# fanxiaochen/Multi-View-Registration

Measured on NVIDIA B200. Metric: nn_queries_per_s (24-view x 200k turntable registration; ms_per_step = registration ms; a query = one PCL-equivalent nearest-neighbour answer: every source point per iteration + every gated match's reciprocal answer, the oracle's counter), higher is better.
Workload: dtype f32

## Files before the change

multi-view-registration_b200/csrc/api.cu:

```cuda
#include <cfloat>
#include <chrono>
#include <cstdlib>
#include <climits>
#include <cmath>
#include <cstdio>
#include <cstring>
#include <memory>
#include <string>
#include <thread>
#include <vector>

#include "../../include/mvr_b200.h"
#include "launch.h"
#include "small_solve.h"

#ifndef MVR_PG_XRATIO
#define MVR_PG_XRATIO 4
#endif

using namespace mvr;

#include <atomic>
namespace mvr {
static std::atomic<unsigned long long> g_launches{0};
void count_launch(int n) { g_launches.fetch_add((unsigned long long)n, std::memory_order_relaxed); }
unsigned long long launch_count() { return g_launches.load(std::memory_order_relaxed); }
}

namespace {

struct DevBuf {
  void* p = nullptr;
  size_t cap = 0;
  cudaError_t ensure(size_t bytes) {
    if (bytes <= cap) return cudaSuccess;
    if (p) cudaFree(p);
    p = nullptr; cap = 0;
    size_t want = bytes + bytes / 8 + 256;
    cudaError_t e = cudaMalloc(&p, want);
    if (e == cudaSuccess) cap = want;
    return e;
  }
  void release() { if (p) cudaFree(p); p = nullptr; cap = 0; }
  template <class T> T* as() const { return (T*)p; }
};

struct Cloud {
  const float4* pts = nullptr;
  DevBuf own;
  int n = 0;
  float lo[3] = {0, 0, 0}, hi[3] = {0, 0, 0};
  int n_bad = 0;
  uint64_t gen = 0;
  bool index_valid = false;
  bool exportable = false;
  uint64_t index_gen = 0;
  mvr_grid grid{};
  GridDev gd{};
  DevBuf keys, vals, keys_alt, vals_alt, hist, counters, sorted, table;
  uint32_t* sorted_keys = nullptr;
  uint32_t* perm = nullptr;
  IndexDev dev() const {
    IndexDev ix;
    ix.pts = sorted.as<float4>(); ix.start = table.as<uint32_t>(); ix.g = gd; ix.n_valid = n - n_bad;
    return ix;
  }
  void release() {
    own.release(); keys.release(); vals.release(); keys_alt.release(); vals_alt.release(); hist.release();
    counters.release(); sorted.release(); table.release();
  }
};

struct ProfRec { int kind; cudaEvent_t a, b; double bytes, units; int count; };

struct PairIndex {
  DevBuf sorted, start, s0;
  DevBuf gocc, gmask;
  float gm_gate = -1.f;
  int gm_stride = 0;
  PairGrid g{};
  uint32_t cells = 0;
  int n_valid = 0;
  uint64_t gen = 0;
  bool valid = false;
  void release() { sorted.release(); start.release(); s0.release(); gocc.release(); gmask.release(); gm_gate = -1.f; valid = false; }
};

}

struct mvr_ctx {
  int device = 0;
  cudaStream_t stream = nullptr;
  bool own_stream = false;
  Cloud tgt, src;
  DevBuf normals; bool has_normals = false;
  DevBuf cur, corr_p, corr_j, corr_d2, rmin, rnn, partials, sums, out_cloud, qtmp, itmp, ftmp, scratch, misc, tiles, state, log;
  PairIndex pt, ps;
  PairIndex nt, nq;
  double nn_ppc = 8.0;
  double nn_dense_ratio = 8.0;
  int nn_mode = MVR_NN_AUTO;
  int nn_sorted_from = 262144;
  bool gate_mask = false;
  FwdArgs fa{}; RevArgs ra{};
  bool want_rnn = false;
  int group_pairs = 0;
  struct BuildScratch { DevBuf keys, vals, moved, count, tiles; uint32_t epoch = 1; } bs[2];
  DevBuf stage_dev;
  IcpState* h_stage = nullptr;
  int stage_cap = 0;
  DevBuf bbox_dev;
  uint32_t* h_bbox = nullptr;
  int log_pending = 0;
  bool out_pending = false;
  DevBuf crowded;
  uint32_t crowded_seen = 0;
  IcpState* h_state = nullptr;
  IterRec* h_log = nullptr;
  double* h_sums = nullptr;
  uint32_t* h_small = nullptr;
  std::string err;
  bool profiling = false;
  std::vector<ProfRec> prof;
  std::vector<cudaEvent_t> ev_pool;
  mvr_kernel_stat stats[MVR_K_COUNT] = {};
  std::vector<mvr_icp_iteration> iters;
  bool have_out = false;
  float cell_edge_opt = 0.f;
  int max_bits_opt = 8;
  cudaEvent_t ev_a = nullptr, ev_b = nullptr;
};

namespace {

#define CK(expr)                                                                                 \
  do {                                                                                           \
    cudaError_t _e = (expr);                                                                     \
    if (_e != cudaSuccess) {                                                                     \
      ctx->err = std::string(#expr) + ": " + cudaGetErrorString(_e);                             \
      return MVR_ERR_CUDA;                                                                       \
    }                                                                                            \
  } while (0)

int fail(mvr_ctx* ctx, int code, const char* msg) {
  if (ctx) ctx->err = msg;
  return code;
}

cudaEvent_t get_event(mvr_ctx* ctx) {
  if (!ctx->ev_pool.empty()) { cudaEvent_t e = ctx->ev_pool.back(); ctx->ev_pool.pop_back(); return e; }
  cudaEvent_t e = nullptr;
  cudaEventCreate(&e);
  return e;
}

struct ProfScope {
  mvr_ctx* ctx; int idx;
  cudaStream_t st;
  ProfScope(mvr_ctx* c, int kind, double bytes, double units, int count = 1, cudaStream_t stream = nullptr) : ctx(c), idx(-1), st(stream ? stream : c->stream) {
    if (!c->profiling) return;
    ProfRec r{kind, get_event(c), get_event(c), bytes, units, count};
    cudaEventRecord(r.a, st);
    c->prof.push_back(r);
    idx = (int)c->prof.size() - 1;
  }
  ~ProfScope() { if (idx >= 0) cudaEventRecord(ctx->prof[idx].b, st); }
};

void prof_flush(mvr_ctx* ctx) {
  for (ProfRec& r : ctx->prof) {
    cudaEventSynchronize(r.b);
    float ms = 0.f;
    if (cudaEventElapsedTime(&ms, r.a, r.b) == cudaSuccess) {
      mvr_kernel_stat& s = ctx->stats[r.kind];
      s.launches += (uint64_t)r.count; s.ms += ms; s.bytes += r.bytes; s.units += r.units;
    }
    ctx->ev_pool.push_back(r.a); ctx->ev_pool.push_back(r.b);
  }
  ctx->prof.clear();
}

double density_cell_edge(const float lo[3], const float hi[3], int n, double ppc) {
  double ex = std::max(0.0, (double)hi[0] - lo[0]), ey = std::max(0.0, (double)hi[1] - lo[1]), ez = std::max(0.0, (double)hi[2] - lo[2]);
  double area = ex * ey + ey * ez + ex * ez;
  double ext = std::max(ex, std::max(ey, ez));
  if (n <= 0 || ext <= 0) return 1.0;
  if (area <= 0) return ext / std::min(1024.0, std::max(1.0, (double)n / ppc));
  return std::sqrt(1.5 * ppc * area / (double)n);
}

mvr_grid make_grid(const float lo[3], const float hi[3], double cell, int max_bits) {
  mvr_grid g{};
  double ext = 0;
  for (int a = 0; a < 3; ++a) ext = std::max(ext, (double)hi[a] - (double)lo[a]);
  if (!(ext > 0) || !std::isfinite(ext)) ext = 1.0;
  if (!(cell > 0) || !std::isfinite(cell)) cell = ext;
  if (max_bits > 10) max_bits = 10;
  if (max_bits < 1) max_bits = 1;
  int bits = std::min(3, max_bits);
  while (bits < max_bits && cell * (double)(1 << bits) < ext * 1.0001) ++bits;
  if (cell * (double)(1 << bits) < ext * 1.0001) cell = ext * 1.0001 / (double)(1 << bits);
  for (int a = 0; a < 3; ++a) g.origin[a] = lo[a];
  g.inv_cell = (float)(1.0 / cell);
  g.cell = (float)cell;
  g.bits = bits;
  return g;
}

GridDev to_dev(const mvr_grid& g) {
  GridDev d;
  d.ox = g.origin[0]; d.oy = g.origin[1]; d.oz = g.origin[2];
  d.inv_cell = g.inv_cell;
  double c = (1.0 / (double)g.inv_cell) * (1.0 - 1e-6);
  d.cell_lo = std::nextafterf((float)c, 0.0f);
  d.bits = g.bits;
  d.G = 1 << g.bits;
  return d;
}

bool same_grid(const mvr_grid& a, const mvr_grid& b) {
  return std::memcmp(a.origin, b.origin, sizeof(a.origin)) == 0 && a.inv_cell == b.inv_cell && a.bits == b.bits;
}

int cloud_bbox(mvr_ctx* ctx, Cloud& c) {
  for (int a = 0; a < 3; ++a) { c.lo[a] = 0; c.hi[a] = 0; }
  c.n_bad = 0;
  if (c.n <= 0) return MVR_OK;
  CK(ctx->misc.ensure(64));
  uint32_t* d = ctx->misc.as<uint32_t>();
  CK(launch_bbox_init(d, ctx->stream));
  CK(launch_bbox(c.pts, c.n, d, ctx->stream));
  CK(cudaMemcpyAsync(ctx->h_small, d, 7 * sizeof(uint32_t), cudaMemcpyDeviceToHost, ctx->stream));
  CK(cudaStreamSynchronize(ctx->stream));
  c.n_bad = (int)ctx->h_small[6];
  if (c.n_bad < c.n)
    for (int a = 0; a < 3; ++a) { c.lo[a] = bbox_decode(ctx->h_small[a]); c.hi[a] = bbox_decode(ctx->h_small[3 + a]); }
  return MVR_OK;
}

int cloud_set(mvr_ctx* ctx, Cloud& c, const float* xyzw, size_t n, bool device_ptr) {
  if (n > (size_t)INT_MAX / 2) return fail(ctx, MVR_ERR_BAD_ARG, "cloud too large");
  if (n > 0 && !xyzw) return fail(ctx, MVR_ERR_BAD_ARG, "null point pointer");
  c.index_valid = false;
  c.gen++;
  c.n = (int)n;
  if (device_ptr) {
    c.pts = (const float4*)xyzw;
  } else {
    CK(c.own.ensure(std::max<size_t>(n, 1) * sizeof(float4)));
    if (n) CK(cudaMemcpyAsync(c.own.p, xyzw, n * sizeof(float4), cudaMemcpyHostToDevice, ctx->stream));
    c.pts = c.own.as<float4>();
  }
  return cloud_bbox(ctx, c);
}

int build_index(mvr_ctx* ctx, Cloud& c, const float4* pts, const mvr_grid& g) {
  const int n = c.n;
  const size_t cells = (size_t)1 << (3 * g.bits);
  CK(c.keys.ensure(std::max(n, 1) * sizeof(uint32_t)));
  CK(c.vals.ensure(std::max(n, 1) * sizeof(uint32_t)));
  CK(c.keys_alt.ensure(std::max(n, 1) * sizeof(uint32_t)));
  CK(c.vals_alt.ensure(std::max(n, 1) * sizeof(uint32_t)));
  CK(c.hist.ensure((size_t)256 * radix_num_blocks(n) * sizeof(uint32_t)));
  CK(c.sorted.ensure(std::max(n, 1) * sizeof(float4)));
  CK(c.table.ensure((cells + 2) * sizeof(uint32_t)));
  c.grid = g;
  c.gd = to_dev(g);
  {
    ProfScope ps(ctx, MVR_K_MORTON, 24.0 * n, n);
    CK(launch_morton_keys(pts, n, c.gd, c.keys.as<uint32_t>(), c.vals.as<uint32_t>(), ctx->stream));
  }
  int key_bits = 3 * g.bits + (c.n_bad > 0 ? 1 : 0);
  SortScratch sc{c.keys_alt.as<uint32_t>(), c.vals_alt.as<uint32_t>(), c.hist.as<uint32_t>()};
  {
    ProfScope ps(ctx, MVR_K_SORT, 16.0 * n, n);
    CK(launch_radix_sort(c.keys.as<uint32_t>(), c.vals.as<uint32_t>(), n, key_bits, sc, &c.sorted_keys, &c.perm, ctx->stream));
  }
  {
    ProfScope ps(ctx, MVR_K_TABLE, 36.0 * n + 4.0 * (double)cells, n);
    CK(launch_gather_sorted(pts, c.perm, n, c.sorted.as<float4>(), ctx->stream));
    CK(launch_cell_table(c.sorted_keys, n, g.bits, c.table.as<uint32_t>(), ctx->stream));
  }
  c.index_valid = true;
  c.exportable = true;
  c.index_gen = c.gen;
  return MVR_OK;
}

mvr_grid auto_grid(mvr_ctx* ctx, const Cloud& c) {
  double e = ctx->cell_edge_opt > 0 ? ctx->cell_edge_opt : density_cell_edge(c.lo, c.hi, c.n - c.n_bad, 6.0);
  return make_grid(c.lo, c.hi, e, ctx->max_bits_opt);
}

PairGrid make_pair_grid(const float lo[3], const float hi[3], double e, uint32_t* cells_out, int xr = 1);
bool same_pair_grid(const PairGrid& a, const PairGrid& b);
int build_pair_index(mvr_ctx* ctx, PairIndex& ix, const float4* pts, int n, int n_bad, const Mat4f* guess, const PairGrid& g,
                     uint32_t cells, bool keep_s0, bool ordered = true);
int plan_pair_index(mvr_ctx* ctx, PairIndex& ix, int slot, const float4* pts, int n, int n_bad, const Mat4f* guess, const PairGrid& g,
                    uint32_t cells, bool ordered, cudaStream_t stream, BuildJob* job);
int run_pair_builds(mvr_ctx* ctx, const BuildJob* jobs, int count, cudaStream_t stream);

double pair_cell_edge(mvr_ctx* ctx, const Cloud& c, double max_dist);

int nn_pass_dense(mvr_ctx* ctx, const float4* q, int n, int32_t* d_idx, float* d_d2, bool seeded) {
  Cloud& t = ctx->tgt;
  const int mv = t.n - t.n_bad;
  const double e = ctx->cell_edge_opt > 0 ? ctx->cell_edge_opt : density_cell_edge(t.lo, t.hi, mv, ctx->nn_ppc);
  uint32_t cells = 0;
  const PairGrid g = make_pair_grid(t.lo, t.hi, e, &cells);
  int rc;
  if (!(ctx->nt.valid && ctx->nt.gen == t.gen && same_pair_grid(ctx->nt.g, g))) {
    if ((rc = build_pair_index(ctx, ctx->nt, t.pts, t.n, t.n_bad, nullptr, g, cells, false))) return rc;
    ctx->nt.gen = t.gen;
  }
  if ((rc = build_pair_index(ctx, ctx->nq, q, n, 0, nullptr, g, cells, false, false))) return rc;
  ProfScope ps(ctx, MVR_K_NN, 24.0 * n + 16.0 * t.n, (double)n);
  if (seeded)
    CK(launch_seeded_nn(ctx->nq.sorted.as<float4>(), n, ctx->nq.start.as<uint32_t>() + cells, ctx->nt.sorted.as<float4>(),
                        ctx->nt.start.as<uint32_t>(), g, mv, d_idx, d_d2, ctx->stream));
  else
    CK(launch_cell_nn(ctx->nq.sorted.as<float4>(), n, ctx->nq.start.as<uint32_t>() + cells, ctx->nt.sorted.as<float4>(),
                      ctx->nt.start.as<uint32_t>(), g, mv, d_idx, d_d2, ctx->stream));
  return MVR_OK;
}

int nn_pass(mvr_ctx* ctx, const float4* q, int n, int32_t* d_idx, float* d_d2) {
  if (ctx->nn_mode == MVR_NN_CELL) return nn_pass_dense(ctx, q, n, d_idx, d_d2, false);
  if (ctx->nn_mode == MVR_NN_SEEDED || (ctx->nn_mode == MVR_NN_AUTO && n > ctx->nn_sorted_from)) return nn_pass_dense(ctx, q, n, d_idx, d_d2, true);
  Cloud& t = ctx->tgt;
  PairIndex& pt = ctx->pt;
  int rc;
  if (!(pt.valid && pt.gen == t.gen && pt.g.xr == 1.0f)) {
    uint32_t cells = 0;
    const PairGrid gt = make_pair_grid(t.lo, t.hi, pair_cell_edge(ctx, t, INFINITY), &cells);
    if ((rc = build_pair_index(ctx, pt, t.pts, t.n, t.n_bad, nullptr, gt, cells, false))) return rc;
    pt.gen = t.gen;
  }
  ProfScope ps(ctx, MVR_K_NN, 24.0 * n + 16.0 * t.n, (double)n);
  if (ctx->nn_mode == MVR_NN_WARP || (ctx->nn_mode == MVR_NN_AUTO && n <= 131072)) {
    CK(launch_warp_nn(q, n, pt.sorted.as<float4>(), pt.start.as<uint32_t>(), pt.g, pt.n_valid, d_idx, d_d2, ctx->stream));
    return MVR_OK;
  }
  const bool sorted = n > 262144;
  if (sorted && (rc = build_pair_index(ctx, ctx->nq, q, n, 0, nullptr, pt.g, pt.cells, false, false))) return rc;
  CK(launch_pair_nn(sorted ? ctx->nq.sorted.as<float4>() : q, n, sorted, pt.sorted.as<float4>(), pt.start.as<uint32_t>(), pt.g, pt.n_valid, d_idx,
                    d_d2, ctx->stream));
  return MVR_OK;
}

void mat_identity(float* m) { for (int k = 0; k < 16; ++k) m[k] = (k % 5 == 0) ? 1.f : 0.f; }

float gate_float(double max_dist) {
  double m2 = max_dist * max_dist;
  if (!(m2 < (double)FLT_MAX)) return INFINITY;
  float f = (float)m2;
  if ((double)f < m2) f = std::nextafterf(f, INFINITY);
  return std::nextafterf(f, INFINITY);
}

double pair_cell_edge(mvr_ctx* ctx, const Cloud& c, double max_dist) {
  if (ctx->cell_edge_opt > 0) return ctx->cell_edge_opt;
  const int nv = c.n - c.n_bad;
  const double e_lo = density_cell_edge(c.lo, c.hi, nv, 2.0), e_hi = density_cell_edge(c.lo, c.hi, nv, 12.0);
  const double m2 = max_dist * max_dist;
  return (m2 < 1e30) ? std::min(std::max(0.5 * max_dist * 1.002, e_lo), e_hi) : density_cell_edge(c.lo, c.hi, nv, 6.0);
}

PairGrid make_pair_grid(const float lo[3], const float hi[3], double e, uint32_t* cells_out, int xr) {
  const double max_cells = 16.0 * 1024 * 1024;
  if (xr != 1 && xr != 2 && xr != 4 && xr != 8) xr = 1;
  double ext[3];
  for (int a = 0; a < 3; ++a) {
    ext[a] = (double)hi[a] - (double)lo[a];
    if (!(ext[a] >= 0) || !std::isfinite(ext[a])) ext[a] = 0;
  }
  if (!(e > 0) || !std::isfinite(e)) e = std::max(1e-3, std::max(ext[0], std::max(ext[1], ext[2])));
  int n[3];
  for (;;) {
    double tot = 1;
    for (int a = 0; a < 3; ++a) {
      const int r = a == 0 ? xr : 1;
      n[a] = (int)std::min(4096.0 * r, std::floor(ext[a] / (e / r)) + 3.0 * r);
      tot *= n[a];
    }
    if (tot <= max_cells) break;
    if (xr > 1) { xr /= 2; continue; }
    e *= 1.25;
  }
  PairGrid g;
  g.ox = lo[0] - (float)e; g.oy = lo[1] - (float)e; g.oz = lo[2] - (float)e;
  if (!std::isfinite(g.ox)) g.ox = 0.f;
  if (!std::isfinite(g.oy)) g.oy = 0.f;
  if (!std::isfinite(g.oz)) g.oz = 0.f;
  g.inv_cell = (float)(1.0 / e);
  g.cell_lo = std::nextafterf((float)((1.0 / (double)g.inv_cell) * (1.0 - 1e-6)), 0.0f);
  g.nx = n[0]; g.ny = n[1]; g.nz = n[2];
  g.xr = (float)xr;
  g.inv_cell_x = g.inv_cell * g.xr;
  *cells_out = (uint32_t)n[0] * (uint32_t)n[1] * (uint32_t)n[2];
  return g;
}

bool same_pair_grid(const PairGrid& a, const PairGrid& b) { return std::memcmp(&a, &b, sizeof(PairGrid)) == 0; }

int plan_pair_index(mvr_ctx* ctx, PairIndex& ix, int slot, const float4* pts, int n, int n_bad, const Mat4f* guess, const PairGrid& g,
                    uint32_t cells, bool ordered, cudaStream_t stream, BuildJob* job) {
  mvr_ctx::BuildScratch& bs = ctx->bs[slot];
  const size_t nn = (size_t)std::max(n, 1);
  CK(bs.keys.ensure(nn * sizeof(uint32_t)));
  CK(bs.vals.ensure(nn * sizeof(uint32_t)));
  if (ordered) CK(bs.moved.ensure(nn * sizeof(float4)));
  CK(ix.sorted.ensure(nn * sizeof(float4)));
  CK(ix.start.ensure(((size_t)cells + 2) * sizeof(uint32_t)));
  if (((size_t)cells + 1) * sizeof(uint32_t) > bs.count.cap) {
    CK(bs.count.ensure(((size_t)cells + 1) * sizeof(uint32_t)));
    CK(cudaMemsetAsync(bs.count.p, 0, bs.count.cap, stream));
  }
  const int ntiles = scan_num_tiles((size_t)cells + 1);
  const size_t tiles = (size_t)ntiles + 1;
  if (tiles * sizeof(unsigned long long) > bs.tiles.cap) {
    CK(bs.tiles.ensure(tiles * sizeof(unsigned long long)));
    CK(cudaMemsetAsync(bs.tiles.p, 0, bs.tiles.cap, stream));
  }
  if (!ctx->crowded.p) { CK(ctx->crowded.ensure(64)); CK(cudaMemsetAsync(ctx->crowded.p, 0, 64, stream)); }
  BuildJob& j = *job;
  j = BuildJob{};
  j.in = pts; j.n = n; j.apply = guess ? 1 : 0;
  if (guess) j.M = *guess;
  j.g = g; j.cells = cells;
  j.keys = bs.keys.as<uint32_t>(); j.rank = bs.vals.as<uint32_t>(); j.counters = bs.count.as<uint32_t>();
  j.tiles = bs.tiles.as<unsigned long long>(); j.epoch = bs.epoch; j.ntiles = ntiles;
  bs.epoch = (bs.epoch % 0x3fffffffu) + 1;
  j.tmp = ordered ? bs.moved.as<float4>() : nullptr; j.sorted = ix.sorted.as<float4>(); j.start = ix.start.as<uint32_t>();
  j.crowded = ctx->crowded.as<uint32_t>(); j.ordered = ordered ? 1 : 0;
  ix.g = g; ix.cells = cells; ix.n_valid = n - n_bad; ix.valid = true; ix.gm_gate = -1.f;
  return MVR_OK;
}

int run_pair_builds(mvr_ctx* ctx, const BuildJob* jobs, int count, cudaStream_t stream) {
  for (int k0 = 0; k0 < count; k0 += BUILD_MAX_JOBS) {
    const int c = std::min(count - k0, (int)BUILD_MAX_JOBS);
    BuildBatch batch;
    double bytes = 0, pts = 0;
    for (int k = 0; k < c; ++k) { batch.j[k] = jobs[k0 + k]; bytes += 32.0 * jobs[k0 + k].n + 8.0 * jobs[k0 + k].cells; pts += jobs[k0 + k].n; }
    ProfScope ps(ctx, MVR_K_SORT, bytes, pts, 1, stream);
    CK(launch_pair_builds(batch, c, stream));
  }
  return MVR_OK;
}

int build_pair_index(mvr_ctx* ctx, PairIndex& ix, const float4* pts, int n, int n_bad, const Mat4f* guess, const PairGrid& g,
                     uint32_t cells, bool keep_s0, bool ordered) {
  (void)keep_s0;
  BuildJob job;
  ix.valid = false;
  int rc = plan_pair_index(ctx, ix, &ix == &ctx->pt || &ix == &ctx->nt ? 0 : 1, pts, n, n_bad, guess, g, cells, ordered, ctx->stream, &job);
  if (rc) { ix.valid = false; return rc; }
  return run_pair_builds(ctx, &job, 1, ctx->stream);
}

int ensure_gate_mask(mvr_ctx* ctx, PairIndex& ix, float max_d2f, cudaStream_t stream) {
  if (!ctx->gate_mask || !(max_d2f < 3.0e38f) || ix.n_valid <= 0) { ix.gm_gate = -1.f; return MVR_OK; }
  if (ix.gm_gate == max_d2f) return MVR_OK;
  const double slack = 2.0 * ((double)MVR_CELL_MARGIN + 1.0e-6 * (double)std::max(ix.g.nx, std::max(ix.g.ny, ix.g.nz)));
  const double need = std::sqrt((double)max_d2f) * (1.0 + 1.0e-5) / (double)ix.g.cell_lo + slack;
  const int D = (int)std::ceil(need);
  const int Dx = (int)std::ceil(need * (double)ix.g.xr);
  ix.gm_gate = -1.f;
  if (D < 1 || D > 6 || Dx > 31) return MVR_OK;
  const int wstride = (ix.g.nx + 31) / 32;
  const size_t words = (size_t)ix.g.ny * ix.g.nz * wstride;
  CK(ix.gocc.ensure(words * sizeof(uint32_t)));
  CK(ix.gmask.ensure(words * sizeof(uint32_t)));
  CK(launch_gate_mask(ix.start.as<uint32_t>(), ix.g, wstride, D, Dx, ix.gocc.as<uint32_t>(), ix.gmask.as<uint32_t>(), stream));
  ix.gm_stride = wstride;
  ix.gm_gate = max_d2f;
  return MVR_OK;
}

int ensure_pinned(mvr_ctx* ctx) {
  if (!ctx->h_sums) CK(cudaMallocHost((void**)&ctx->h_sums, REDUCE_MAX_VALS * sizeof(double)));
  if (!ctx->h_small) CK(cudaMallocHost((void**)&ctx->h_small, 64 * sizeof(uint32_t)));
  if (!ctx->h_state) CK(cudaMallocHost((void**)&ctx->h_state, sizeof(IcpState)));
  if (!ctx->h_log) CK(cudaMallocHost((void**)&ctx->h_log, ICP_MAX_LOG * sizeof(IterRec)));
  return MVR_OK;
}

template <class F>
void parallel_for(int n, F fn) {
  static const int max_threads = [] { const char* e = std::getenv("MVR_HOST_THREADS"); const int v = e ? std::atoi(e) : 6; return v < 1 ? 1 : (v > 64 ? 64 : v); }();
  const int nt = std::min(max_threads, n);
  if (nt <= 1) { for (int k = 0; k < n; ++k) fn(k); return; }
  std::atomic<int> next{0};
  auto work = [&] { for (int k = next.fetch_add(1); k < n; k = next.fetch_add(1)) fn(k); };
  std::vector<std::thread> th;
  for (int t = 1; t < nt; ++t) th.emplace_back(work);
  work();
  for (std::thread& t : th) t.join();
}

PairGrid normals_grid(const mvr_ctx* ctx, const Cloud& c, int k, uint32_t* cells) {
  const double e = ctx->cell_edge_opt > 0 ? ctx->cell_edge_opt : density_cell_edge(c.lo, c.hi, c.n - c.n_bad, std::max(2.0, k / 3.0));
  return make_pair_grid(c.lo, c.hi, e, cells);
}

NormalsJob normals_job(const PairIndex& ix, int n, const float* viewpoint, float4* out, int32_t* nbr) {
  NormalsJob j{};
  j.sorted = ix.sorted.as<float4>(); j.start = ix.start.as<uint32_t>(); j.g = ix.g;
  j.n = n; j.n_valid = ix.n_valid;
  j.viewpoint = viewpoint ? make_float3(viewpoint[0], viewpoint[1], viewpoint[2]) : make_float3(0.f, 0.f, 0.f);
  j.out = out; j.nbr = nbr;
  return j;
}


}

extern "C" {

const char* mvr_version(void) { return "mvr_b200 0.1 (sm_100a)"; }

uint64_t mvr_kernel_launch_count(void) { return (uint64_t)launch_count(); }

void mvr_transfer_sizes(size_t* state_bytes, size_t* log_record_bytes) {
  if (state_bytes) *state_bytes = sizeof(IcpState);
  if (log_record_bytes) *log_record_bytes = sizeof(IterRec);
}

const char* mvr_status_string(int s) {
  switch (s) {
    case MVR_OK: return "ok";
    case MVR_ERR_BAD_ARG: return "bad argument";
    case MVR_ERR_TOO_FEW_CORRESPONDENCES: return "not enough correspondences";
    case MVR_ERR_CUDA: return "CUDA error";
    case MVR_ERR_NO_INPUT: return "input cloud not set";
    case MVR_ERR_NOT_SPD: return "normal equations not positive definite";
    case MVR_ERR_ALLOC: return "allocation failed";
    case MVR_ERR_NCCL: return "NCCL unavailable or a collective failed";
    default: return "unknown status";
  }
}

void mvr_icp_params_default(mvr_icp_params* p) {
  if (!p) return;
  p->max_iterations = 10;
  p->max_correspondence_distance = std::sqrt(DBL_MAX);
  p->transformation_epsilon = 0.0;
  p->euclidean_fitness_epsilon = -DBL_MAX;
  p->use_reciprocal_correspondences = 0;
  p->estimator = MVR_POINT_TO_POINT;
  p->fixed_iterations = 0;
  p->min_correspondences = 3;
}

int mvr_ctx_create(int device, mvr_ctx** out) {
  if (!out) return MVR_ERR_BAD_ARG;
  *out = nullptr;
  int count = 0;
  if (cudaGetDeviceCount(&count) != cudaSuccess || count <= 0 || device < 0 || device >= count) return MVR_ERR_CUDA;
  if (cudaSetDevice(device) != cudaSuccess) return MVR_ERR_CUDA;
  mvr_ctx* ctx = new mvr_ctx();
  ctx->device = device;
  if (cudaStreamCreateWithFlags(&ctx->stream, cudaStreamNonBlocking) != cudaSuccess) { delete ctx; return MVR_ERR_CUDA; }
  ctx->own_stream = true;
  cudaEventCreate(&ctx->ev_a);
  cudaEventCreate(&ctx->ev_b);
  if (ensure_pinned(ctx) != MVR_OK) { mvr_ctx_destroy(ctx); return MVR_ERR_CUDA; }
  *out = ctx;
  return MVR_OK;
}

int mvr_ctx_destroy(mvr_ctx* ctx) {
  if (!ctx) return MVR_OK;
  cudaSetDevice(ctx->device);
  cudaStreamSynchronize(ctx->stream);
  prof_flush(ctx);
  for (cudaEvent_t e : ctx->ev_pool) cudaEventDestroy(e);
  if (ctx->ev_a) cudaEventDestroy(ctx->ev_a);
  if (ctx->ev_b) cudaEventDestroy(ctx->ev_b);
  ctx->tgt.release(); ctx->src.release(); ctx->normals.release();
  ctx->pt.release(); ctx->ps.release(); ctx->nt.release(); ctx->nq.release();
  for (auto& b : ctx->bs) { b.keys.release(); b.vals.release(); b.moved.release(); b.count.release(); b.tiles.release(); }
  ctx->stage_dev.release(); ctx->bbox_dev.release();
  if (ctx->h_stage) cudaFreeHost(ctx->h_stage);
  if (ctx->h_bbox) cudaFreeHost(ctx->h_bbox);
  DevBuf* bufs[] = {&ctx->cur, &ctx->corr_p, &ctx->rmin, &ctx->rnn, &ctx->corr_j, &ctx->corr_d2, &ctx->partials, &ctx->sums, &ctx->out_cloud, &ctx->qtmp,
                    &ctx->itmp, &ctx->ftmp, &ctx->scratch, &ctx->misc, &ctx->tiles, &ctx->state, &ctx->log, &ctx->crowded};
  for (DevBuf* b : bufs) b->release();
  if (ctx->h_sums) cudaFreeHost(ctx->h_sums);
  if (ctx->h_small) cudaFreeHost(ctx->h_small);
  if (ctx->h_state) cudaFreeHost(ctx->h_state);
  if (ctx->h_log) cudaFreeHost(ctx->h_log);
  if (ctx->own_stream && ctx->stream) cudaStreamDestroy(ctx->stream);
  delete ctx;
  return MVR_OK;
}

int mvr_ctx_set_stream(mvr_ctx* ctx, void* s) {
  if (!ctx) return MVR_ERR_BAD_ARG;
  cudaSetDevice(ctx->device);
  cudaStreamSynchronize(ctx->stream);
  if (ctx->own_stream && ctx->stream) cudaStreamDestroy(ctx->stream);
  ctx->stream = (cudaStream_t)s;
  ctx->own_stream = false;
  return MVR_OK;
}

void* mvr_ctx_get_stream(mvr_ctx* ctx) { return ctx ? (void*)ctx->stream : nullptr; }

int mvr_ctx_synchronize(mvr_ctx* ctx) {
  if (!ctx) return MVR_ERR_BAD_ARG;
  CK(cudaStreamSynchronize(ctx->stream));
  return MVR_OK;
}

const char* mvr_last_error(mvr_ctx* ctx) { return ctx ? ctx->err.c_str() : "null context"; }

int mvr_ctx_set_profiling(mvr_ctx* ctx, int on) {
  if (!ctx) return MVR_ERR_BAD_ARG;
  ctx->profiling = on != 0;
  return MVR_OK;
}

int mvr_ctx_get_kernel_stats(mvr_ctx* ctx, mvr_kernel_stat* out, int reset) {
  if (!ctx || !out) return MVR_ERR_BAD_ARG;
  cudaSetDevice(ctx->device);
  CK(cudaStreamSynchronize(ctx->stream));
  prof_flush(ctx);
  std::memcpy(out, ctx->stats, sizeof(ctx->stats));
  if (reset) std::memset(ctx->stats, 0, sizeof(ctx->stats));
  return MVR_OK;
}

int mvr_ctx_set_index_options(mvr_ctx* ctx, float cell_edge, int max_bits) {
  if (!ctx) return MVR_ERR_BAD_ARG;
  if (max_bits < 1 || max_bits > 10) return fail(ctx, MVR_ERR_BAD_ARG, "max_bits must be in 1..10");
  ctx->cell_edge_opt = cell_edge > 0 ? cell_edge : 0.f;
  ctx->max_bits_opt = max_bits;
  ctx->tgt.index_valid = false;
  ctx->src.index_valid = false;
  return MVR_OK;
}

int mvr_ctx_set_nn_options(mvr_ctx* ctx, double points_per_cell, double dense_ratio) {
  if (!ctx || !(points_per_cell > 0) || !(dense_ratio >= 0)) return MVR_ERR_BAD_ARG;
  ctx->nn_ppc = points_per_cell;
  ctx->nn_dense_ratio = dense_ratio;
  ctx->nt.valid = false;
  return MVR_OK;
}

int mvr_ctx_set_gate_mask(mvr_ctx* ctx, int on) {
  if (!ctx) return MVR_ERR_BAD_ARG;
  ctx->gate_mask = on != 0;
  ctx->pt.gm_gate = -1.f;
  return MVR_OK;
}

int mvr_ctx_set_nn_mode(mvr_ctx* ctx, int mode) {
  if (!ctx || mode < MVR_NN_AUTO || mode > MVR_NN_SEEDED) return MVR_ERR_BAD_ARG;
  ctx->nn_mode = mode;
  return MVR_OK;
}

int mvr_ctx_set_batch_group(mvr_ctx* ctx, int pairs) {
  if (!ctx || pairs < 0 || pairs > (int)FUSED_MAX_PAIRS) return MVR_ERR_BAD_ARG;
  ctx->group_pairs = pairs;
  return MVR_OK;
}

int mvr_set_target(mvr_ctx* ctx, const float* xyzw, size_t n) {
  if (!ctx) return MVR_ERR_BAD_ARG;
  cudaSetDevice(ctx->device);
  ctx->has_normals = false;
  return cloud_set(ctx, ctx->tgt, xyzw, n, false);
}
int mvr_set_source(mvr_ctx* ctx, const float* xyzw, size_t n) {
  if (!ctx) return MVR_ERR_BAD_ARG;
  cudaSetDevice(ctx->device);
  ctx->have_out = false;
  return cloud_set(ctx, ctx->src, xyzw, n, false);
}
int mvr_set_target_device(mvr_ctx* ctx, const float* d, size_t n) {
  if (!ctx) return MVR_ERR_BAD_ARG;
  cudaSetDevice(ctx->device);
  ctx->has_normals = false;
  return cloud_set(ctx, ctx->tgt, d, n, true);
}
int mvr_set_source_device(mvr_ctx* ctx, const float* d, size_t n) {
  if (!ctx) return MVR_ERR_BAD_ARG;
  cudaSetDevice(ctx->device);
  ctx->have_out = false;
  return cloud_set(ctx, ctx->src, d, n, true);
}

int mvr_set_clouds_device(mvr_ctx* const* ctxs, const int* which, const float* const* d_xyzw, const size_t* n, int count) {
  if (count < 0 || (count && (!ctxs || !which || !d_xyzw || !n))) return MVR_ERR_BAD_ARG;
  if (count == 0) return MVR_OK;
  mvr_ctx* ctx = ctxs[0];
  if (!ctx) return MVR_ERR_BAD_ARG;
  for (int k = 0; k < count; ++k) {
    if (!ctxs[k] || (which[k] != MVR_CLOUD_TARGET && which[k] != MVR_CLOUD_SOURCE)) return MVR_ERR_BAD_ARG;
    if (ctxs[k]->device != ctx->device) return fail(ctx, MVR_ERR_BAD_ARG, "the contexts of a batch must share a device");
    if (n[k] > (size_t)INT_MAX / 2) return fail(ctx, MVR_ERR_BAD_ARG, "cloud too large");
    if (n[k] > 0 && !d_xyzw[k]) return fail(ctx, MVR_ERR_BAD_ARG, "null point pointer");
  }
  cudaSetDevice(ctx->device);
  if (!ctx->h_bbox) CK(cudaMallocHost((void**)&ctx->h_bbox, (size_t)BBOX_MAX_JOBS * 7 * sizeof(uint32_t)));
  CK(ctx->bbox_dev.ensure((size_t)BBOX_MAX_JOBS * 7 * sizeof(uint32_t)));
  for (int k0 = 0; k0 < count; k0 += BBOX_MAX_JOBS) {
    const int c = std::min(count - k0, (int)BBOX_MAX_JOBS);
    BboxBatch bb;
    for (int k = 0; k < c; ++k) { bb.j[k].pts = (const float4*)d_xyzw[k0 + k]; bb.j[k].n = (int)n[k0 + k]; bb.j[k].pad_ = 0; }
    CK(launch_bbox_batch(bb, c, ctx->bbox_dev.as<uint32_t>(), ctx->stream));
    CK(cudaMemcpyAsync(ctx->h_bbox, ctx->bbox_dev.p, (size_t)c * 7 * sizeof(uint32_t), cudaMemcpyDeviceToHost, ctx->stream));
    CK(cudaStreamSynchronize(ctx->stream));
    for (int k = 0; k < c; ++k) {
      mvr_ctx* m = ctxs[k0 + k];
      Cloud& cl = which[k0 + k] == MVR_CLOUD_TARGET ? m->tgt : m->src;
      if (which[k0 + k] == MVR_CLOUD_TARGET) m->has_normals = false; else { m->have_out = false; m->out_pending = false; }
      cl.index_valid = false;
      cl.gen++;
      cl.n = (int)n[k0 + k];
      cl.pts = (const float4*)d_xyzw[k0 + k];
      const uint32_t* w = ctx->h_bbox + 7 * k;
      for (int a = 0; a < 3; ++a) { cl.lo[a] = 0; cl.hi[a] = 0; }
      cl.n_bad = cl.n > 0 ? (int)w[6] : 0;
      if (cl.n > 0 && cl.n_bad < cl.n)
        for (int a = 0; a < 3; ++a) { cl.lo[a] = bbox_decode(w[a]); cl.hi[a] = bbox_decode(w[3 + a]); }
    }
  }
  return MVR_OK;
}

int mvr_cloud_share(mvr_ctx* dst, int which_dst, mvr_ctx* src, int which_src) {
  if (!dst || !src || (which_dst != MVR_CLOUD_TARGET && which_dst != MVR_CLOUD_SOURCE) ||
      (which_src != MVR_CLOUD_TARGET && which_src != MVR_CLOUD_SOURCE)) return MVR_ERR_BAD_ARG;
  if (dst->device != src->device) return fail(dst, MVR_ERR_BAD_ARG, "contexts on different devices");
  const Cloud& s = which_src == MVR_CLOUD_TARGET ? src->tgt : src->src;
  Cloud& d = which_dst == MVR_CLOUD_TARGET ? dst->tgt : dst->src;
  if (s.gen == 0) return fail(dst, MVR_ERR_NO_INPUT, "cloud not set");
  if (&s == &d) return MVR_OK;
  d.index_valid = false;
  d.gen++;
  d.pts = s.pts; d.n = s.n; d.n_bad = s.n_bad;
  for (int a = 0; a < 3; ++a) { d.lo[a] = s.lo[a]; d.hi[a] = s.hi[a]; }
  if (which_dst == MVR_CLOUD_TARGET) dst->has_normals = false; else dst->have_out = false;
  return MVR_OK;
}

int mvr_set_target_normals(mvr_ctx* ctx, const float* nxyzc, size_t n) {
  if (!ctx || !nxyzc) return MVR_ERR_BAD_ARG;
  cudaSetDevice(ctx->device);
  if ((int)n != ctx->tgt.n) return fail(ctx, MVR_ERR_BAD_ARG, "normals count differs from target size");
  CK(ctx->normals.ensure(std::max<size_t>(n, 1) * sizeof(float4)));
  CK(cudaMemcpyAsync(ctx->normals.p, nxyzc, n * sizeof(float4), cudaMemcpyHostToDevice, ctx->stream));
  CK(cudaStreamSynchronize(ctx->stream));
  ctx->has_normals = true;
  return MVR_OK;
}

int mvr_get_bbox(mvr_ctx* ctx, int which, float lo[3], float hi[3]) {
  if (!ctx || !lo || !hi || (which != MVR_CLOUD_TARGET && which != MVR_CLOUD_SOURCE)) return MVR_ERR_BAD_ARG;
  const Cloud& c = which == MVR_CLOUD_TARGET ? ctx->tgt : ctx->src;
  if (c.gen == 0) return fail(ctx, MVR_ERR_NO_INPUT, "cloud not set");
  for (int a = 0; a < 3; ++a) { lo[a] = c.lo[a]; hi[a] = c.hi[a]; }
  return MVR_OK;
}

int mvr_index_build(mvr_ctx* ctx, int which, const mvr_grid* grid) {
  if (!ctx || (which != MVR_CLOUD_TARGET && which != MVR_CLOUD_SOURCE)) return MVR_ERR_BAD_ARG;
  cudaSetDevice(ctx->device);
  Cloud& c = which == MVR_CLOUD_TARGET ? ctx->tgt : ctx->src;
  if (!c.pts && c.n == 0 && c.gen == 0) return fail(ctx, MVR_ERR_NO_INPUT, "cloud not set");
  mvr_grid g;
  if (grid) {
    if (grid->bits < 1 || grid->bits > 10 || !(grid->inv_cell > 0)) return fail(ctx, MVR_ERR_BAD_ARG, "bad grid");
    g = *grid;
  } else {
    g = auto_grid(ctx, c);
  }
  return build_index(ctx, c, c.pts, g);
}

int mvr_index_export(mvr_ctx* ctx, int which, mvr_grid* grid, uint32_t* sorted_keys, int32_t* perm, uint32_t* cell_start) {
  if (!ctx || (which != MVR_CLOUD_TARGET && which != MVR_CLOUD_SOURCE)) return MVR_ERR_BAD_ARG;
  cudaSetDevice(ctx->device);
  Cloud& c = which == MVR_CLOUD_TARGET ? ctx->tgt : ctx->src;
  if (!c.index_valid || !c.exportable) return fail(ctx, MVR_ERR_NO_INPUT, "index not built (call mvr_index_build first)");
  if (grid) *grid = c.grid;
  if (sorted_keys && c.n) CK(cudaMemcpyAsync(sorted_keys, c.sorted_keys, c.n * sizeof(uint32_t), cudaMemcpyDeviceToHost, ctx->stream));
  if (perm && c.n) CK(cudaMemcpyAsync(perm, c.perm, c.n * sizeof(uint32_t), cudaMemcpyDeviceToHost, ctx->stream));
  if (cell_start) CK(cudaMemcpyAsync(cell_start, c.table.p, (((size_t)1 << (3 * c.grid.bits)) + 1) * sizeof(uint32_t), cudaMemcpyDeviceToHost, ctx->stream));
  CK(cudaStreamSynchronize(ctx->stream));
  return MVR_OK;
}

int mvr_nn_query_device(mvr_ctx* ctx, const float* d_q, size_t n, int32_t* d_idx, float* d_d2) {
  if (!ctx || (n && (!d_q || !d_idx || !d_d2))) return MVR_ERR_BAD_ARG;
  if (n > (size_t)INT_MAX / 2) return fail(ctx, MVR_ERR_BAD_ARG, "too many queries");
  cudaSetDevice(ctx->device);
  if (ctx->tgt.gen == 0) return fail(ctx, MVR_ERR_NO_INPUT, "target not set");
  if (n == 0) return MVR_OK;
  return nn_pass(ctx, (const float4*)d_q, (int)n, d_idx, d_d2);
}

int mvr_nn_query(mvr_ctx* ctx, const float* q, size_t n, int32_t* idx, float* d2) {
  if (!ctx || (n && (!q || !idx || !d2))) return MVR_ERR_BAD_ARG;
  cudaSetDevice(ctx->device);
  if (ctx->tgt.gen == 0) return fail(ctx, MVR_ERR_NO_INPUT, "target not set");
  if (n == 0) return MVR_OK;
  CK(ctx->qtmp.ensure(n * sizeof(float4)));
  CK(ctx->itmp.ensure(n * sizeof(int32_t)));
  CK(ctx->ftmp.ensure(n * sizeof(float)));
  CK(cudaMemcpyAsync(ctx->qtmp.p, q, n * sizeof(float4), cudaMemcpyHostToDevice, ctx->stream));
  int rc = mvr_nn_query_device(ctx, ctx->qtmp.as<float>(), n, ctx->itmp.as<int32_t>(), ctx->ftmp.as<float>());
  if (rc) return rc;
  CK(cudaMemcpyAsync(idx, ctx->itmp.p, n * sizeof(int32_t), cudaMemcpyDeviceToHost, ctx->stream));
  CK(cudaMemcpyAsync(d2, ctx->ftmp.p, n * sizeof(float), cudaMemcpyDeviceToHost, ctx->stream));
  CK(cudaStreamSynchronize(ctx->stream));
  return MVR_OK;
}

static int align_prepare_batch(mvr_ctx* const* ctxs, int count, const mvr_icp_params* prm, const float* guesses, int est, int* statuses,
                               std::vector<mvr_ctx*>& ok, std::vector<int>& slot);
static int align_prepare(mvr_ctx* ctx, const mvr_icp_params* prm, const float* guess, int est) {
  int st = MVR_OK;
  std::vector<mvr_ctx*> ok;
  std::vector<int> slot;
  const int rc = align_prepare_batch(&ctx, 1, prm, guess, est, &st, ok, slot);
  return rc ? rc : st;
}

static int align_run(mvr_ctx* const* ctxs, int count, const mvr_icp_params* prm, int est);

int mvr_correspondences(mvr_ctx* ctx, double max_dist, int reciprocal, int32_t* iq, int32_t* im, float* dist, size_t* count) {
  if (!ctx || !count) return MVR_ERR_BAD_ARG;
  cudaSetDevice(ctx->device);
  *count = 0;
  if (ctx->tgt.gen == 0 || ctx->src.gen == 0) return fail(ctx, MVR_ERR_NO_INPUT, "source/target not set");
  if (!(max_dist >= 0)) return fail(ctx, MVR_ERR_BAD_ARG, "max_dist must be >= 0");
  const int n = ctx->src.n;
  if (n == 0 || ctx->tgt.n == 0) return MVR_OK;
  if (!iq || !im || !dist) return MVR_ERR_BAD_ARG;
  mvr_icp_params one;
  mvr_icp_params_default(&one);
  one.max_iterations = 1; one.fixed_iterations = 1;
  one.use_reciprocal_correspondences = reciprocal ? 1 : 0;
  one.max_correspondence_distance = max_dist;
  one.min_correspondences = 1;
  ctx->want_rnn = true;
  int rc = align_prepare(ctx, &one, nullptr, EST_P2P);
  ctx->want_rnn = false;
  if (rc) return rc;
  if ((rc = align_run(&ctx, 1, &one, EST_P2P))) return rc;
  if (ctx->h_state->dbg[2] != 0) return fail(ctx, MVR_ERR_CUDA, "internal error: a reciprocal search lost its chooser (search bound violated)");
  CK(ctx->corr_j.ensure((size_t)n * sizeof(int32_t)));
  CK(ctx->corr_d2.ensure((size_t)n * sizeof(float)));
  CK(ctx->scratch.ensure(compact_scratch_elems(n) * sizeof(uint32_t) + 64));
  CK(ctx->itmp.ensure((size_t)2 * n * sizeof(int32_t)));
  CK(ctx->ftmp.ensure((size_t)n * sizeof(float)));
  CK(ctx->misc.ensure(64));
  int32_t* dq = ctx->itmp.as<int32_t>();
  int32_t* dm = dq + n;
  CK(cudaMemsetAsync(ctx->corr_j.p, 0xff, (size_t)n * sizeof(int32_t), ctx->stream));
  CK(launch_resolve_pairs(ctx->fa.cur, ctx->fa.n_valid, ctx->fa.corr_p, ctx->ra.rnn, ctx->fa.tgt, ctx->corr_j.as<int32_t>(),
                          ctx->corr_d2.as<float>(), ctx->stream));
  CK(launch_compact_corr(ctx->corr_j.as<int32_t>(), ctx->corr_d2.as<float>(), n, ctx->scratch.as<uint32_t>(), dq, dm,
                         ctx->ftmp.as<float>(), ctx->misc.as<uint32_t>(), ctx->stream));
  CK(cudaMemcpyAsync(ctx->h_small, ctx->misc.p, sizeof(uint32_t), cudaMemcpyDeviceToHost, ctx->stream));
  CK(cudaStreamSynchronize(ctx->stream));
  size_t c = ctx->h_small[0];
  if (c) {
    CK(cudaMemcpyAsync(iq, dq, c * sizeof(int32_t), cudaMemcpyDeviceToHost, ctx->stream));
    CK(cudaMemcpyAsync(im, dm, c * sizeof(int32_t), cudaMemcpyDeviceToHost, ctx->stream));
    CK(cudaMemcpyAsync(dist, ctx->ftmp.p, c * sizeof(float), cudaMemcpyDeviceToHost, ctx->stream));
    CK(cudaStreamSynchronize(ctx->stream));
  }
  *count = c;
  return MVR_OK;
}

static int align_plan(mvr_ctx* ctx, const mvr_icp_params* prm, const float* guess, int est, cudaStream_t S, std::vector<BuildJob>& jobs) {
  cudaSetDevice(ctx->device);
  if (ctx->tgt.gen == 0 || ctx->src.gen == 0) return fail(ctx, MVR_ERR_NO_INPUT, "source/target not set");
  Cloud& s = ctx->src;
  const int n = s.n;
  if (n == 0 || ctx->tgt.n == 0) return fail(ctx, MVR_ERR_NO_INPUT, "empty source or target");
  if (prm->estimator == MVR_POINT_TO_PLANE && !ctx->has_normals)
    return fail(ctx, MVR_ERR_NO_INPUT, "point-to-plane needs target normals (mvr_set_target_normals / mvr_estimate_normals)");
  if (!(prm->max_correspondence_distance >= 0)) return fail(ctx, MVR_ERR_BAD_ARG, "max_correspondence_distance");
  float G[16];
  if (guess) std::memcpy(G, guess, sizeof(G)); else mat_identity(G);
  const bool reciprocal = prm->use_reciprocal_correspondences != 0;
  const double max_dist = prm->max_correspondence_distance;
  const bool p2l = est == EST_P2L;

  const int m = ctx->tgt.n;
  int rc = MVR_OK;
  {
    uint32_t cells = 0;
    const PairGrid gt = make_pair_grid(ctx->tgt.lo, ctx->tgt.hi, pair_cell_edge(ctx, ctx->tgt, max_dist), &cells, MVR_PG_XRATIO);
    PairIndex& pt = ctx->pt;
    if (!(pt.valid && pt.gen == ctx->tgt.gen && same_pair_grid(pt.g, gt))) {
      BuildJob job;
      pt.valid = false;
      if ((rc = plan_pair_index(ctx, pt, 0, ctx->tgt.pts, m, ctx->tgt.n_bad, nullptr, gt, cells, true, S, &job))) { pt.valid = false; return rc; }
      jobs.push_back(job);
      pt.gen = ctx->tgt.gen;
    }
  }
  {
    float lo[3] = {INFINITY, INFINITY, INFINITY}, hi[3] = {-INFINITY, -INFINITY, -INFINITY};
    if (s.n - s.n_bad > 0) {
      for (int corner = 0; corner < 8; ++corner) {
        const double p[3] = {(corner & 1) ? s.hi[0] : s.lo[0], (corner & 2) ? s.hi[1] : s.lo[1], (corner & 4) ? s.hi[2] : s.lo[2]};
        for (int a = 0; a < 3; ++a) {
          const double v = G[a] * p[0] + G[4 + a] * p[1] + G[8 + a] * p[2] + G[12 + a];
          if (std::isfinite(v)) { lo[a] = std::min(lo[a], (float)v); hi[a] = std::max(hi[a], (float)v); }
        }
      }
    }
    for (int a = 0; a < 3; ++a) if (!(lo[a] <= hi[a])) { lo[a] = 0.f; hi[a] = 0.f; }
    uint32_t cells = 0;
    const PairGrid gs = make_pair_grid(lo, hi, pair_cell_edge(ctx, s, max_dist), &cells, MVR_PG_XRATIO);
    Mat4f Gm;
    std::memcpy(Gm.m, G, sizeof(Gm.m));
    BuildJob job;
    ctx->ps.valid = false;
    if ((rc = plan_pair_index(ctx, ctx->ps, 1, s.pts, n, s.n_bad, &Gm, gs, cells, true, S, &job))) { ctx->ps.valid = false; return rc; }
    jobs.push_back(job);
    for (int a = 0; a < 3; ++a) { ctx->h_state->box[a] = lo[a]; ctx->h_state->box[3 + a] = hi[a]; }
  }
  const PairIndex &pt = ctx->pt, &psx = ctx->ps;
  CK(ctx->corr_p.ensure((size_t)std::max(n, 1) * sizeof(int32_t)));
  if (reciprocal) CK(ctx->rmin.ensure((size_t)std::max(m, 1) * sizeof(uint32_t)));
  CK(ctx->partials.ensure((size_t)std::max((int)FUSED_MAX_BLOCKS, fused_grid_rev(m)) * REDUCE_MAX_VALS * sizeof(double)));
  CK(ctx->state.ensure(sizeof(IcpState)));
  CK(ctx->log.ensure((size_t)ICP_MAX_LOG * sizeof(IterRec)));
  IcpState* d_st = ctx->state.as<IcpState>();
  IterRec* d_log = ctx->log.as<IterRec>();

  IcpState& h = *ctx->h_state;
  double sbox[6];
  for (int a = 0; a < 6; ++a) sbox[a] = h.box[a];
  std::memset(&h, 0, sizeof(h));
  for (int a = 0; a < 3; ++a) {
    const double pad = 1e-3 + 1e-5 * std::max(std::fabs(sbox[a]), std::fabs(sbox[3 + a]));
    h.box[a] = sbox[a] - pad; h.box[3 + a] = sbox[3 + a] + pad;
    h.babs[a] = std::max(std::fabs(h.box[a]), std::fabs(h.box[3 + a]));
  }
  h.devd = 0.0; h.dev = 0.0f;
  for (int k = 0; k < 16; ++k) { h.delta[k] = (k % 5 == 0) ? 1.f : 0.f; h.fin[k] = G[k]; h.cum[k] = (k % 5 == 0) ? 1.0 : 0.0; }
  for (int k = 0; k < 12; ++k) h.cinv[k] = (k % 5 == 0) ? 1.0 : 0.0;
  h.stretch = 1.0f;
  h.prev_mse = DBL_MAX;
  h.rot_thr = 1.0 - prm->transformation_epsilon;
  h.trans_thr = prm->transformation_epsilon;
  h.fit_eps = prm->euclidean_fitness_epsilon;
  h.ox = 0.5 * ((double)ctx->tgt.lo[0] + ctx->tgt.hi[0]);
  h.oy = 0.5 * ((double)ctx->tgt.lo[1] + ctx->tgt.hi[1]);
  h.oz = 0.5 * ((double)ctx->tgt.lo[2] + ctx->tgt.hi[2]);
  h.max_iter = prm->max_iterations;
  h.fixed = prm->fixed_iterations != 0;
  h.min_corr = prm->min_correspondences > 0 ? prm->min_correspondences : 3;
  h.p2l = p2l; h.recip = reciprocal; h.n_src = n;
  if (prm->max_iterations <= 0) { h.done = 1; h.reason = MVR_REASON_ITERATIONS; }
  ctx->iters.clear();
  ctx->log_pending = 0;
  ctx->have_out = false; ctx->out_pending = false;

  FwdArgs& fa = ctx->fa;
  fa = FwdArgs{};
  fa.cur = psx.sorted.as<float4>(); fa.n_valid = psx.n_valid;
  fa.tgt = pt.sorted.as<float4>(); fa.tstart = pt.start.as<uint32_t>(); fa.gt = pt.g; fa.m_valid = pt.n_valid;
  fa.corr_p = ctx->corr_p.as<int32_t>(); fa.rmin = reciprocal ? ctx->rmin.as<uint32_t>() : nullptr;
  fa.max2 = max_dist * max_dist; fa.max_d2f = gate_float(max_dist);
  fa.gmask = nullptr; fa.gm_stride = 0;
  fa.nrm = p2l ? ctx->normals.as<float4>() : nullptr;
  fa.partials = ctx->partials.as<double>(); fa.st = d_st; fa.log = d_log; fa.grid = fused_grid(psx.n_valid);
  RevArgs& ra = ctx->ra;
  ra = RevArgs{};
  ra.tgt = fa.tgt; ra.m_valid = pt.n_valid; ra.rmin = fa.rmin; ra.cur = fa.cur; ra.sstart = psx.start.as<uint32_t>(); ra.gs = psx.g;
  ra.n_valid = psx.n_valid; ra.corr_p = fa.corr_p; ra.nrm = fa.nrm;
  ra.rnn = nullptr;
  if (reciprocal && ctx->want_rnn) { CK(ctx->rnn.ensure((size_t)std::max(m, 1) * sizeof(int32_t))); ra.rnn = ctx->rnn.as<int32_t>(); }
  ra.partials = fa.partials; ra.st = d_st; ra.log = d_log; ra.grid = fused_grid_rev(pt.n_valid); ra.per = fused_rev_chunks(pt.n_valid);
  return MVR_OK;
}

static int ensure_stage(mvr_ctx* lead, int count) {
  mvr_ctx* ctx = lead;
  if (count > lead->stage_cap) {
    if (lead->h_stage) cudaFreeHost(lead->h_stage);
    lead->h_stage = nullptr; lead->stage_cap = 0;
    const int want = std::max(count + count / 2, 8);
    CK(cudaMallocHost((void**)&lead->h_stage, (size_t)want * sizeof(IcpState)));
    lead->stage_cap = want;
  }
  CK(lead->stage_dev.ensure((size_t)lead->stage_cap * sizeof(IcpState)));
  return MVR_OK;
}

static InitJob init_job_of(mvr_ctx* c) {
  InitJob j{};
  j.corr_p = c->corr_p.as<int32_t>(); j.n = std::max(c->src.n, 1); j.m = std::max(c->tgt.n, 1);
  j.rmin = c->fa.rmin; j.st = c->state.as<IcpState>(); j.crowded = c->crowded.as<uint32_t>();
  return j;
}

static int batch_group_size(const mvr_ctx* lead, int count) {
  return lead->group_pairs > 0 ? std::min(lead->group_pairs, (int)FUSED_MAX_PAIRS) : std::max(1, std::min((count + 3) / 4, (int)FUSED_MAX_PAIRS));
}

static int align_prepare_batch(mvr_ctx* const* ctxs, int count, const mvr_icp_params* prm, const float* guesses, int est, int* statuses,
                               std::vector<mvr_ctx*>& ok, std::vector<int>& slot) {
  ok.clear(); slot.clear();
  if (count <= 0) return MVR_OK;
  const int gsz0 = batch_group_size(ctxs[0], count);
  std::vector<std::vector<BuildJob>> jobs((size_t)count);
  for (int k = 0; k < count; ++k) if (ensure_pinned(ctxs[k]) != MVR_OK) return MVR_ERR_CUDA;
  parallel_for(count, [&](int k) {
    statuses[k] = align_plan(ctxs[k], prm, guesses ? guesses + 16 * k : nullptr, est, ctxs[(k / gsz0) * gsz0]->stream, jobs[(size_t)k]);
  });
  for (int k = 0; k < count; ++k)
    if (statuses[k] == MVR_OK) { ok.push_back(ctxs[k]); slot.push_back(k); }
  if (ok.empty()) return MVR_OK;
  mvr_ctx* ctx = ok[0];
  const int P = (int)ok.size();
  const int gsz = batch_group_size(ctx, P);
  if (P != count || gsz != gsz0) {
    for (int k = 0; k < count; k += gsz0) {
      cudaEvent_t e = ctxs[k]->ev_b;
      CK(cudaEventRecord(e, ctxs[k]->stream));
      for (int g0 = 0; g0 < P; g0 += gsz) CK(cudaStreamWaitEvent(ok[(size_t)g0]->stream, e, 0));
    }
  }
  int rc = ensure_stage(ctx, P);
  if (rc) return rc;
  for (int g0 = 0; g0 < P; g0 += gsz) {
    const int gn = std::min(gsz, P - g0);
    cudaStream_t S = ok[(size_t)g0]->stream;
    std::vector<BuildJob> all;
    for (int k = 0; k < gn; ++k) { const std::vector<BuildJob>& j = jobs[(size_t)slot[(size_t)(g0 + k)]]; all.insert(all.end(), j.begin(), j.end()); }
    if ((rc = run_pair_builds(ctx, all.data(), (int)all.size(), S))) return rc;
    for (int k0 = 0; k0 < gn; k0 += BUILD_MAX_JOBS) {
      const int c = std::min(gn - k0, (int)BUILD_MAX_JOBS);
      InitBatch ib;
      for (int k = 0; k < c; ++k) {
        mvr_ctx* m = ok[(size_t)(g0 + k0 + k)];
        ib.j[k] = init_job_of(m);
        std::memcpy(ctx->h_stage + g0 + k0 + k, m->h_state, sizeof(IcpState));
      }
      CK(cudaMemcpyAsync(ctx->stage_dev.as<IcpState>() + g0 + k0, ctx->h_stage + g0 + k0, (size_t)c * sizeof(IcpState), cudaMemcpyHostToDevice, S));
      CK(launch_align_init(ib, c, ctx->stage_dev.as<IcpState>() + g0 + k0, S));
    }
    for (int k = 0; k < gn; ++k) {
      mvr_ctx* m = ok[(size_t)(g0 + k)];
      if ((rc = ensure_gate_mask(m, m->pt, m->fa.max_d2f, S))) { ctx->err = m->err; return rc; }
      m->fa.gmask = m->pt.gm_gate >= 0.f ? m->pt.gmask.as<uint32_t>() : nullptr; m->fa.gm_stride = m->pt.gm_stride;
    }
  }
  return MVR_OK;
}

static int align_run(mvr_ctx* const* ctxs, int count, const mvr_icp_params* prm, int est) {
  mvr_ctx* ctx = ctxs[0];
  cudaSetDevice(ctx->device);
  const bool reciprocal = prm->use_reciprocal_correspondences != 0;
  const int gsz = batch_group_size(ctx, count);
  struct Group {
    int g0, gn, gf, gr, enqueued, first, todo;
    bool done, fetched;
    long long n_tot, m_tot;
    mvr_ctx* lead;
    FwdBatch fb;
    RevBatch rb;
  };
  long long batch_points = 0;
  for (int k = 0; k < count; ++k) batch_points += ctxs[k]->fa.n_valid;
  static const int fwd_items_env = [] { const char* e = std::getenv("MVR_FWD_ITEMS"); return e ? std::atoi(e) : 0; }();
  const int fwd_items = fwd_items_env > 0 ? fwd_items_env : (int)std::min<long long>(4, std::max<long long>(1, (batch_points + 300000) / 600000));
  std::vector<Group> groups;
  for (int g0 = 0; g0 < count; g0 += gsz) {
    Group g{};
    g.g0 = g0; g.gn = std::min(gsz, count - g0); g.gf = 1; g.gr = 1; g.enqueued = 0; g.first = 1; g.done = true; g.fetched = true;
    g.lead = ctxs[g0];
    for (int k = 0; k < g.gn; ++k) {
      mvr_ctx* c = ctxs[g0 + k];
      g.fb.a[k] = c->fa; g.rb.a[k] = c->ra;
      if (reciprocal && fwd_items > 1) g.fb.a[k].grid = std::max(1, (c->fa.n_valid + FUSED_THREADS * fwd_items - 1) / (FUSED_THREADS * fwd_items));
      g.gf = std::max(g.gf, g.fb.a[k].grid); g.gr = std::max(g.gr, c->ra.grid);
      if (!c->h_state->done) g.done = false;
      g.n_tot += c->src.n; g.m_tot += c->tgt.n;
    }
    groups.push_back(g);
  }
  int rc0 = ensure_stage(ctx, count);
  if (rc0) return rc0;
  if (ctx->profiling) {
    for (Group& g : groups) CK(cudaStreamSynchronize(g.lead->stream));
    CK(cudaEventRecord(ctx->ev_a, ctx->stream));
    for (size_t gi = 1; gi < groups.size(); ++gi) CK(cudaStreamWaitEvent(groups[gi].lead->stream, ctx->ev_a, 0));
  } else {
    CK(cudaEventRecord(ctx->ev_a, ctx->stream));
  }
  auto unpack = [&](Group& g) {
    if (g.fetched) return;
    g.fetched = true;
    for (int k = 0; k < g.gn; ++k) {
      mvr_ctx* c = ctxs[g.g0 + k];
      std::memcpy(c->h_state, ctx->h_stage + g.g0 + k, sizeof(IcpState));
      c->crowded_seen = std::max(c->crowded_seen, (uint32_t)c->h_state->dbg[3]);
      c->h_state->dbg[3] = 0;
    }
  };
  for (int k = 0; k < count; ++k) ctxs[k]->crowded_seen = 0;
  int batch = prm->fixed_iterations ? 64 : 2;
  for (;;) {
    bool any = false;
    int todo_max = 0;
    std::vector<std::unique_ptr<ProfScope>> scopes;
    for (Group& g : groups) {
      g.todo = 0;
      if (g.done) continue;
      any = true;
      g.todo = std::min(batch, std::max(prm->max_iterations - g.enqueued, 1));
      todo_max = std::max(todo_max, g.todo);
      const double per_it = 16.0 * g.n_tot + 16.0 * g.m_tot + (reciprocal ? 52.0 * g.n_tot : 0.0);
      scopes.emplace_back(new ProfScope(g.lead, MVR_K_CORR, per_it * g.todo, (double)g.n_tot * g.todo, g.todo));
    }
    for (int it = 0; it < todo_max; ++it)
      for (Group& g : groups) {
        if (it >= g.todo) continue;
        CK(launch_icp_forward(g.fb, g.gn, g.gf, g.first, reciprocal, est, g.lead->stream));
        g.first = 0;
        if (reciprocal) CK(launch_icp_reverse(g.rb, g.gn, g.gr, est, g.lead->stream));
      }
    scopes.clear();
    for (Group& g : groups) {
      if (g.todo == 0) continue;
      g.enqueued += g.todo;
      for (int k0 = 0; k0 < g.gn; k0 += BUILD_MAX_JOBS) {
        const int c = std::min(g.gn - k0, (int)BUILD_MAX_JOBS);
        InitBatch ib;
        for (int k = 0; k < c; ++k) ib.j[k] = init_job_of(ctxs[g.g0 + k0 + k]);
        IcpState* d = ctx->stage_dev.as<IcpState>() + g.g0 + k0;
        CK(launch_align_gather(ib, c, d, g.lead->stream));
        CK(cudaMemcpyAsync(ctx->h_stage + g.g0 + k0, d, (size_t)c * sizeof(IcpState), cudaMemcpyDeviceToHost, g.lead->stream));
      }
      g.fetched = false;
    }
    if (!any) break;
    bool more = false;
    for (Group& g : groups) {
      if (g.done) continue;
      if (prm->fixed_iterations) {
        g.done = g.enqueued >= prm->max_iterations;
      } else {
        CK(cudaStreamSynchronize(g.lead->stream));
        unpack(g);
        g.done = true;
        for (int k = 0; k < g.gn; ++k) if (!ctxs[g.g0 + k]->h_state->done) g.done = false;
      }
      if (!g.done) more = true;
    }
    if (!more) break;
    batch = std::min(batch * 2, 64);
  }
  for (size_t gi = 1; gi < groups.size(); ++gi) {
    CK(cudaEventRecord(groups[gi].lead->ev_a, groups[gi].lead->stream));
    CK(cudaStreamWaitEvent(ctx->stream, groups[gi].lead->ev_a, 0));
  }
  CK(cudaEventRecord(ctx->ev_b, ctx->stream));
  CK(cudaStreamSynchronize(ctx->stream));
  for (Group& g : groups) unpack(g);
  return MVR_OK;
}

static int materialize_out(mvr_ctx* ctx) {
  if (!ctx->have_out || !ctx->out_pending) return MVR_OK;
  const int n = ctx->src.n;
  CK(ctx->out_cloud.ensure((size_t)std::max(n, 1) * sizeof(float4)));
  {
    ProfScope ps(ctx, MVR_K_TRANSFORM, 32.0 * n, n);
    CK(launch_transform_final(ctx->src.pts, ctx->out_cloud.as<float4>(), n, ctx->state.as<IcpState>(), ctx->stream));
  }
  ctx->out_pending = false;
  return MVR_OK;
}

static int fetch_log(mvr_ctx* ctx) {
  const int n_log = ctx->log_pending;
  if (n_log <= 0) return MVR_OK;
  ctx->log_pending = 0;
  CK(cudaMemcpyAsync(ctx->h_log, ctx->log.p, (size_t)n_log * sizeof(IterRec), cudaMemcpyDeviceToHost, ctx->stream));
  CK(cudaStreamSynchronize(ctx->stream));
  for (int k = 0; k < n_log; ++k) {
    mvr_icp_iteration rec;
    rec.iteration = ctx->h_log[k].iteration; rec.n_correspondences = ctx->h_log[k].n_corr; rec.mse = ctx->h_log[k].mse;
    std::memcpy(rec.delta, ctx->h_log[k].delta, sizeof(rec.delta));
    ctx->iters.push_back(rec);
  }
  return MVR_OK;
}

static int align_finish_collect(mvr_ctx* ctx, mvr_ctx* lead, float* out_pose, mvr_icp_report* report, int batch_pairs = 1) {
  const IcpState& h = *ctx->h_state;
  if (h.dbg[2] != 0) return fail(ctx, MVR_ERR_CUDA, "internal error: a reciprocal search lost its chooser (search bound violated)");
  ctx->have_out = true; ctx->out_pending = true;
  ctx->log_pending = std::min(h.iter, (int)ICP_MAX_LOG);
  if (out_pose) for (int k = 0; k < 16; ++k) out_pose[k] = (float)h.fin[k];
  if (report) {
    float ms = 0.f;
    cudaEventElapsedTime(&ms, lead->ev_a, lead->ev_b);
    report->iterations = h.iter; report->converged = (h.done && h.status == 0) ? 1 : 0; report->reason = h.reason;
    report->n_correspondences = h.n_corr; report->mse = h.cur_mse; report->nn_queries = h.queries;
    report->gpu_ms = (double)ms / (double)std::max(batch_pairs, 1);
  }
  if (ctx->crowded_seen)
    ctx->err = "warning: a grid cell holds " + std::to_string(ctx->crowded_seen) + " points (duplicates or clamped outliers?): index build and search slow down, sums over it lose their fixed order";
  if (h.status == MVR_ERR_TOO_FEW_CORRESPONDENCES) ctx->err = "not enough correspondences";
  if (h.status == MVR_ERR_NOT_SPD) ctx->err = "point-to-plane normal equations not positive definite";
  return h.status;
}

static int align_finish(mvr_ctx* ctx, mvr_ctx* lead, float* out_pose, float* out_xyzw, mvr_icp_report* report) {
  const int status = align_finish_collect(ctx, lead, out_pose, report);
  if (out_xyzw && ctx->have_out) {
    int rc = materialize_out(ctx);
    if (rc) return rc;
    CK(cudaMemcpyAsync(out_xyzw, ctx->out_cloud.p, (size_t)ctx->src.n * sizeof(float4), cudaMemcpyDeviceToHost, ctx->stream));
    CK(cudaStreamSynchronize(ctx->stream));
  }
  return status;
}

static int icp_align_impl(mvr_ctx* ctx, const mvr_icp_params* prm, const float* guess, float* out_pose, float* out_xyzw,
                          mvr_icp_report* report, bool moments) {
  if (!ctx || !prm) return MVR_ERR_BAD_ARG;
  const bool p2l = prm->estimator == MVR_POINT_TO_PLANE;
  if (moments && p2l) return fail(ctx, MVR_ERR_BAD_ARG, "pair moments are point-to-point statistics");
  const int est = p2l ? EST_P2L : (moments ? EST_MOM : EST_P2P);
  int rc = align_prepare(ctx, prm, guess, est);
  if (rc) return rc;
  if ((rc = align_run(&ctx, 1, prm, est))) return rc;
  return align_finish(ctx, ctx, out_pose, out_xyzw, report);
}

int mvr_icp_align(mvr_ctx* ctx, const mvr_icp_params* prm, const float* guess, float* out_pose, float* out_xyzw,
                  mvr_icp_report* report) {
  return icp_align_impl(ctx, prm, guess, out_pose, out_xyzw, report, false);
}

int mvr_icp_align_batch(mvr_ctx* const* ctxs, int count, const mvr_icp_params* prm, const float* guesses, float* out_poses,
                        mvr_icp_report* reports, int* statuses) {
  if (count < 0 || (count && (!ctxs || !statuses)) || !prm) return MVR_ERR_BAD_ARG;
  if (count == 0) return MVR_OK;
  for (int k = 0; k < count; ++k) {
    if (!ctxs[k]) return MVR_ERR_BAD_ARG;
    for (int j = 0; j < k; ++j) if (ctxs[j] == ctxs[k]) return fail(ctxs[0], MVR_ERR_BAD_ARG, "a context appears twice in the batch");
    if (ctxs[k]->device != ctxs[0]->device) return fail(ctxs[0], MVR_ERR_BAD_ARG, "the contexts of a batch must share a device");
  }
  const int est = prm->estimator == MVR_POINT_TO_PLANE ? EST_P2L : EST_P2P;
  std::vector<mvr_ctx*> ok;
  std::vector<int> slot;
  const bool timing = std::getenv("MVR_DEBUG_TIMING") != nullptr;
  auto now = [] { return std::chrono::duration<double, std::milli>(std::chrono::steady_clock::now().time_since_epoch()).count(); };
  const double t0 = now();
  int rc = align_prepare_batch(ctxs, count, prm, guesses, est, statuses, ok, slot);
  if (rc) { if (!ok.empty() && ok[0] != ctxs[0]) ctxs[0]->err = ok[0]->err; return rc; }
  if (ok.empty()) return MVR_OK;
  const double t1 = now();
  rc = align_run(ok.data(), (int)ok.size(), prm, est);
  if (timing) std::fprintf(stderr, "[timing]   prepare (host enqueue) %.3f ms, run %.3f ms\n", t1 - t0, now() - t1);
  if (rc) { if (ok[0] != ctxs[0]) ctxs[0]->err = ok[0]->err; return rc; }
  for (size_t j = 0; j < ok.size(); ++j) {
    const int k = slot[j];
    statuses[k] = align_finish_collect(ok[j], ok[0], out_poses ? out_poses + 16 * k : nullptr, reports ? reports + k : nullptr, (int)ok.size());
  }
  return MVR_OK;
}

int mvr_pair_moments_compute(mvr_ctx* ctx, double max_dist, int reciprocal, const float* guess, mvr_pair_moments* out) {
  if (!ctx || !out) return MVR_ERR_BAD_ARG;
  std::memset(out, 0, sizeof(*out));
  mvr_icp_params one;
  mvr_icp_params_default(&one);
  one.max_iterations = 1; one.fixed_iterations = 1;
  one.use_reciprocal_correspondences = reciprocal ? 1 : 0;
  one.max_correspondence_distance = max_dist;
  one.min_correspondences = 1;
  mvr_icp_report rep{};
  const int rc = icp_align_impl(ctx, &one, guess, nullptr, nullptr, &rep, true);
  if (rc != MVR_OK && rc != MVR_ERR_TOO_FEW_CORRESPONDENCES) return rc;
  const IcpState& h = *ctx->h_state;
  out->origin[0] = h.ox; out->origin[1] = h.oy; out->origin[2] = h.oz;
  if (rc == MVR_OK) {
    out->n = h.sums[0];
    for (int k = 0; k < 3; ++k) { out->sa[k] = h.sums[1 + k]; out->sb[k] = h.sums[4 + k]; }
    for (int k = 0; k < 9; ++k) out->sba[k] = h.sums[7 + k];
    out->d2 = h.sums[16];
    for (int k = 0; k < 6; ++k) { out->saa[k] = h.sums[17 + k]; out->sbb[k] = h.sums[23 + k]; }
  }
  return MVR_OK;
}

static void moments_from_state(const IcpState& h, bool have, mvr_pair_moments* out) {
  std::memset(out, 0, sizeof(*out));
  out->origin[0] = h.ox; out->origin[1] = h.oy; out->origin[2] = h.oz;
  if (!have) return;
  out->n = h.sums[0];
  for (int k = 0; k < 3; ++k) { out->sa[k] = h.sums[1 + k]; out->sb[k] = h.sums[4 + k]; }
  for (int k = 0; k < 9; ++k) out->sba[k] = h.sums[7 + k];
  out->d2 = h.sums[16];
  for (int k = 0; k < 6; ++k) { out->saa[k] = h.sums[17 + k]; out->sbb[k] = h.sums[23 + k]; }
}

int mvr_pair_moments_compute_batch(mvr_ctx* const* ctxs, int count, double max_dist, int reciprocal, const float* guesses,
                                   mvr_pair_moments* out, int* statuses) {
  if (count < 0 || (count && (!ctxs || !out || !statuses))) return MVR_ERR_BAD_ARG;
  if (count == 0) return MVR_OK;
  for (int k = 0; k < count; ++k) {
    if (!ctxs[k]) return MVR_ERR_BAD_ARG;
    for (int j = 0; j < k; ++j) if (ctxs[j] == ctxs[k]) return fail(ctxs[0], MVR_ERR_BAD_ARG, "a context appears twice in the batch");
    if (ctxs[k]->device != ctxs[0]->device) return fail(ctxs[0], MVR_ERR_BAD_ARG, "the contexts of a batch must share a device");
  }
  mvr_icp_params one;
  mvr_icp_params_default(&one);
  one.max_iterations = 1; one.fixed_iterations = 1;
  one.use_reciprocal_correspondences = reciprocal ? 1 : 0;
  one.max_correspondence_distance = max_dist;
  one.min_correspondences = 1;
  std::vector<mvr_ctx*> ok;
  std::vector<int> slot;
  for (int k = 0; k < count; ++k) std::memset(out + k, 0, sizeof(mvr_pair_moments));
  int rc = align_prepare_batch(ctxs, count, &one, guesses, EST_MOM, statuses, ok, slot);
  if (rc) { if (!ok.empty() && ok[0] != ctxs[0]) ctxs[0]->err = ok[0]->err; return rc; }
  if (ok.empty()) return MVR_OK;
  rc = align_run(ok.data(), (int)ok.size(), &one, EST_MOM);
  if (rc) { if (ok[0] != ctxs[0]) ctxs[0]->err = ok[0]->err; return rc; }
  for (size_t j = 0; j < ok.size(); ++j) {
    const IcpState& h = *ok[j]->h_state;
    const int k = slot[j];
    if (h.dbg[2] != 0) { statuses[k] = fail(ok[j], MVR_ERR_CUDA, "internal error: a reciprocal search lost its chooser (search bound violated)"); continue; }
    const bool have = h.status == MVR_OK;
    statuses[k] = (have || h.status == MVR_ERR_TOO_FEW_CORRESPONDENCES) ? MVR_OK : h.status;
    moments_from_state(h, have, out + k);
    ok[j]->have_out = false; ok[j]->out_pending = false;
  }
  return MVR_OK;
}

double mvr_debug_value(mvr_ctx* ctx, int k) {
  if (ctx && k == 8) return (double)ctx->crowded_seen;
  if (!ctx || !ctx->h_state || k < 0 || k >= 8) return 0.0;
  return (double)ctx->h_state->dbg[k];
}

int mvr_icp_get_iterations(mvr_ctx* ctx, mvr_icp_iteration* out, int max_records, int* count) {
  if (!ctx || !count) return MVR_ERR_BAD_ARG;
  cudaSetDevice(ctx->device);
  int rcl = fetch_log(ctx);
  if (rcl) return rcl;
  int c = (int)ctx->iters.size();
  if (out) {
    int m = std::min(c, std::max(max_records, 0));
    if (m) std::memcpy(out, ctx->iters.data(), (size_t)m * sizeof(mvr_icp_iteration));
    *count = m;
  } else {
    *count = c;
  }
  return MVR_OK;
}

int mvr_fitness_score(mvr_ctx* ctx, double max_range, double* score) {
  if (!ctx || !score) return MVR_ERR_BAD_ARG;
  cudaSetDevice(ctx->device);
  if (ctx->tgt.gen == 0 || ctx->src.gen == 0) return fail(ctx, MVR_ERR_NO_INPUT, "source/target not set");
  const int n = ctx->src.n;
  *score = DBL_MAX;
  if (n == 0 || ctx->tgt.n == 0) return MVR_OK;
  int rc = materialize_out(ctx);
  if (rc) return rc;
  const float4* cloud = ctx->have_out ? ctx->out_cloud.as<float4>() : ctx->src.pts;
  CK(ctx->itmp.ensure((size_t)n * sizeof(int32_t)));
  CK(ctx->ftmp.ensure((size_t)n * sizeof(float)));
  CK(ctx->partials.ensure((size_t)REDUCE_BLOCKS * REDUCE_MAX_VALS * sizeof(double)));
  CK(ctx->sums.ensure(REDUCE_MAX_VALS * sizeof(double)));
  if ((rc = nn_pass(ctx, cloud, n, ctx->itmp.as<int32_t>(), ctx->ftmp.as<float>()))) return rc;
  CK(launch_reduce_fitness(ctx->itmp.as<int32_t>(), ctx->ftmp.as<float>(), n, max_range, ctx->partials.as<double>(),
                           ctx->sums.as<double>(), ctx->stream));
  CK(cudaMemcpyAsync(ctx->h_sums, ctx->sums.p, 2 * sizeof(double), cudaMemcpyDeviceToHost, ctx->stream));
  CK(cudaStreamSynchronize(ctx->stream));
  if (ctx->h_sums[1] > 0) *score = ctx->h_sums[0] / ctx->h_sums[1];
  return MVR_OK;
}

int mvr_apply_pose(mvr_ctx* ctx, const void* points, size_t n, size_t stride_bytes, const double* pose, float* out_xyzw) {
  if (!ctx || !pose || (n && (!points || !out_xyzw))) return MVR_ERR_BAD_ARG;
  if (stride_bytes < 12 || stride_bytes % 4 != 0) return fail(ctx, MVR_ERR_BAD_ARG, "stride must be a multiple of 4 and >= 12");
  if (n > (size_t)INT_MAX / 2) return fail(ctx, MVR_ERR_BAD_ARG, "cloud too large");
  cudaSetDevice(ctx->device);
  if (n == 0) return MVR_OK;
  CK(ctx->scratch.ensure(n * stride_bytes));
  CK(ctx->qtmp.ensure(n * sizeof(float4)));
  CK(cudaMemcpyAsync(ctx->scratch.p, points, n * stride_bytes, cudaMemcpyHostToDevice, ctx->stream));
  CK(launch_apply_pose(ctx->scratch.p, stride_bytes, (int)n, pose, ctx->qtmp.as<float4>(), ctx->stream));
  CK(cudaMemcpyAsync(out_xyzw, ctx->qtmp.p, n * sizeof(float4), cudaMemcpyDeviceToHost, ctx->stream));
  CK(cudaStreamSynchronize(ctx->stream));
  return MVR_OK;
}

int mvr_apply_pose_device(mvr_ctx* ctx, const void* d_points, size_t n, size_t stride_bytes, const double* pose, float* d_out) {
  if (!ctx || !pose || (n && (!d_points || !d_out))) return MVR_ERR_BAD_ARG;
  if (stride_bytes < 12 || stride_bytes % 4 != 0) return fail(ctx, MVR_ERR_BAD_ARG, "stride must be a multiple of 4 and >= 12");
  if (n > (size_t)INT_MAX / 2) return fail(ctx, MVR_ERR_BAD_ARG, "cloud too large");
  cudaSetDevice(ctx->device);
  if (n == 0) return MVR_OK;
  CK(launch_apply_pose(d_points, stride_bytes, (int)n, pose, (float4*)d_out, ctx->stream));
  CK(cudaStreamSynchronize(ctx->stream));
  return MVR_OK;
}

int mvr_merge_registered(mvr_ctx* ctx, const void* const* views, const size_t* counts, const double* poses, const int* registered,
                         int n_views, int full_matrix_normals, void* out, size_t* out_count) {
  if (!ctx || n_views < 0 || !out_count || (n_views && (!views || !counts || !poses))) return MVR_ERR_BAD_ARG;
  cudaSetDevice(ctx->device);
  size_t total = 0;
  for (int v = 0; v < n_views; ++v) {
    if (registered && !registered[v]) continue;
    if (counts[v] && !views[v]) return fail(ctx, MVR_ERR_BAD_ARG, "null view");
    if (counts[v] > (size_t)INT_MAX / 4) return fail(ctx, MVR_ERR_BAD_ARG, "view too large");
    total += counts[v];
  }
  *out_count = total;
  if (!out || total == 0) return MVR_OK;
  CK(ctx->scratch.ensure(total * 48));
  size_t biggest = 0;
  for (int v = 0; v < n_views; ++v) if (!registered || registered[v]) biggest = std::max(biggest, counts[v]);
  CK(ctx->qtmp.ensure(std::max<size_t>(biggest, 1) * 48));
  size_t at = 0;
  for (int v = 0; v < n_views; ++v) {
    if ((registered && !registered[v]) || counts[v] == 0) continue;
    CK(cudaMemcpyAsync(ctx->qtmp.p, views[v], counts[v] * 48, cudaMemcpyHostToDevice, ctx->stream));
    CK(launch_merge_rich(ctx->qtmp.p, (int)counts[v], poses + 16 * v, full_matrix_normals, (char*)ctx->scratch.p + at * 48, ctx->stream));
    at += counts[v];
  }
  CK(cudaMemcpyAsync(out, ctx->scratch.p, total * 48, cudaMemcpyDeviceToHost, ctx->stream));
  CK(cudaStreamSynchronize(ctx->stream));
  return MVR_OK;
}

int mvr_copy_aligned_device(mvr_ctx* ctx, float* d_out) {
  if (!ctx || !d_out) return MVR_ERR_BAD_ARG;
  cudaSetDevice(ctx->device);
  if (!ctx->have_out) return fail(ctx, MVR_ERR_NO_INPUT, "no align has run");
  int rcm = materialize_out(ctx);
  if (rcm) return rcm;
  if (ctx->src.n > 0) CK(cudaMemcpyAsync(d_out, ctx->out_cloud.p, (size_t)ctx->src.n * sizeof(float4), cudaMemcpyDeviceToDevice, ctx->stream));
  CK(cudaStreamSynchronize(ctx->stream));
  return MVR_OK;
}

int mvr_denoise(mvr_ctx* ctx, const void* points, size_t n, size_t stride_bytes, int segment_threshold, double triangle_length,
                int32_t* kept_index, size_t* kept_count, size_t* noise_count) {
  if (!ctx || !kept_count || (n && (!points || !kept_index))) return MVR_ERR_BAD_ARG;
  if (stride_bytes < 12 || stride_bytes % 4 != 0) return fail(ctx, MVR_ERR_BAD_ARG, "stride must be a multiple of 4 and >= 12");
  if (!(triangle_length > 0) || !std::isfinite(triangle_length)) return fail(ctx, MVR_ERR_BAD_ARG, "triangle_length must be positive");
  if (n > (size_t)INT_MAX / 4) return fail(ctx, MVR_ERR_BAD_ARG, "cloud too large");
  cudaSetDevice(ctx->device);
  *kept_count = 0;
  if (noise_count) *noise_count = 0;
  if (n == 0) return MVR_OK;
  const int ni = (int)n;
  CK(ctx->scratch.ensure(n * stride_bytes));
  CK(ctx->qtmp.ensure(n * sizeof(float4)));
  CK(cudaMemcpyAsync(ctx->scratch.p, points, n * stride_bytes, cudaMemcpyHostToDevice, ctx->stream));
  const double I16[16] = {1, 0, 0, 0, 0, 1, 0, 0, 0, 0, 1, 0, 0, 0, 0, 1};
  CK(launch_apply_pose(ctx->scratch.p, stride_bytes, ni, I16, ctx->qtmp.as<float4>(), ctx->stream));
  Cloud tmp;
  tmp.pts = ctx->qtmp.as<float4>(); tmp.n = ni;
  int rc = cloud_bbox(ctx, tmp);
  if (rc) return rc;
  uint32_t cells = 0;
  const PairGrid g = make_pair_grid(tmp.lo, tmp.hi, triangle_length * 1.0001, &cells);
  if ((double)g.cell_lo < triangle_length) return fail(ctx, MVR_ERR_BAD_ARG, "cloud too large for this edge length (grid capped)");
  PairIndex& ix = ctx->nq;
  if ((rc = build_pair_index(ctx, ix, tmp.pts, ni, tmp.n_bad, nullptr, g, cells, false, false))) return rc;
  const size_t nb = (size_t)radix_num_blocks(ni) * 256;
  CK(ctx->itmp.ensure(((size_t)6 * n + nb + 16) * sizeof(uint32_t)));
  uint32_t* parent = ctx->itmp.as<uint32_t>();
  uint32_t *count = parent + n, *keys = count + n, *vals = keys + n, *keys_alt = vals + n, *vals_alt = keys_alt + n, *hist = vals_alt + n, *d_noise = hist + nb;
  CK(cudaMemsetAsync(d_noise, 0, sizeof(uint32_t), ctx->stream));
  CK(launch_denoise_components(ix.sorted.as<float4>(), ix.start.as<uint32_t>(), g, ni, ix.n_valid, triangle_length, parent, keys, count, ctx->stream));
  CK(launch_denoise_keys(count, ni, (uint32_t)std::max(segment_threshold, 0), keys, vals, d_noise, ctx->stream));
  uint32_t *ko = nullptr, *vo = nullptr;
  SortScratch sc{keys_alt, vals_alt, hist};
  CK(launch_radix_sort(keys, vals, ni, 32, sc, &ko, &vo, ctx->stream));
  CK(cudaMemcpyAsync(ctx->h_small, d_noise, sizeof(uint32_t), cudaMemcpyDeviceToHost, ctx->stream));
  CK(cudaStreamSynchronize(ctx->stream));
  const size_t noise = ctx->h_small[0], kept = n - noise;
  if (kept) CK(cudaMemcpyAsync(kept_index, vo, kept * sizeof(uint32_t), cudaMemcpyDeviceToHost, ctx->stream));
  CK(cudaStreamSynchronize(ctx->stream));
  *kept_count = kept;
  if (noise_count) *noise_count = noise;
  ctx->nq.valid = false;
  return MVR_OK;
}

int mvr_estimate_normals(mvr_ctx* ctx, int which, int k, const float viewpoint[3], float* out, int32_t* neighbours) {
  if (!ctx || !out || (which != MVR_CLOUD_TARGET && which != MVR_CLOUD_SOURCE)) return MVR_ERR_BAD_ARG;
  if (k < 3 || k > 32) return fail(ctx, MVR_ERR_BAD_ARG, "k must be in 3..32");
  cudaSetDevice(ctx->device);
  Cloud& c = which == MVR_CLOUD_TARGET ? ctx->tgt : ctx->src;
  if (c.gen == 0) return fail(ctx, MVR_ERR_NO_INPUT, "cloud not set");
  const int n = c.n;
  if (n == 0) return MVR_OK;
  uint32_t cells = 0;
  const PairGrid g = normals_grid(ctx, c, k, &cells);
  PairIndex& ix = ctx->nq;
  int rc = build_pair_index(ctx, ix, c.pts, n, c.n_bad, nullptr, g, cells, false, false);
  if (rc) return rc;
  DevBuf& nb = which == MVR_CLOUD_TARGET ? ctx->normals : ctx->qtmp;
  CK(nb.ensure((size_t)n * sizeof(float4)));
  int32_t* dn = nullptr;
  if (neighbours) { CK(ctx->itmp.ensure((size_t)n * k * sizeof(int32_t))); dn = ctx->itmp.as<int32_t>(); }
  NormalsBatch batch;
  batch.j[0] = normals_job(ix, n, viewpoint, nb.as<float4>(), dn);
  {
    ProfScope ps(ctx, MVR_K_NORMALS, 32.0 * n, n);
    CK(launch_normals(batch, 1, k, ctx->stream));
  }
  ix.valid = false;
  CK(cudaMemcpyAsync(out, nb.p, (size_t)n * sizeof(float4), cudaMemcpyDeviceToHost, ctx->stream));
  if (neighbours) CK(cudaMemcpyAsync(neighbours, dn, (size_t)n * k * sizeof(int32_t), cudaMemcpyDeviceToHost, ctx->stream));
  CK(cudaStreamSynchronize(ctx->stream));
  if (which == MVR_CLOUD_TARGET) ctx->has_normals = true;
  return MVR_OK;
}

int mvr_estimate_normals_batch(mvr_ctx* const* ctxs, int count, int k, const float* viewpoints, float* const* out_nxyzc, int* statuses) {
  if (count < 0 || (count && (!ctxs || !statuses))) return MVR_ERR_BAD_ARG;
  if (count == 0) return MVR_OK;
  for (int a = 0; a < count; ++a) {
    if (!ctxs[a]) return MVR_ERR_BAD_ARG;
    for (int b = 0; b < a; ++b) if (ctxs[b] == ctxs[a]) return fail(ctxs[0], MVR_ERR_BAD_ARG, "a context appears twice in the batch");
    if (ctxs[a]->device != ctxs[0]->device) return fail(ctxs[0], MVR_ERR_BAD_ARG, "the contexts of a batch must share a device");
  }
  mvr_ctx* ctx = ctxs[0];
  if (k < 3 || k > 32) return fail(ctx, MVR_ERR_BAD_ARG, "k must be in 3..32");
  cudaSetDevice(ctx->device);
  const cudaStream_t S = ctx->stream;
  cudaEvent_t ev = get_event(ctx);
  if (!ev) return fail(ctx, MVR_ERR_CUDA, "cudaEventCreate failed");
  struct Todo { mvr_ctx* m; int slot; NormalsJob job; };
  std::vector<Todo> todo;
  std::vector<BuildJob> builds;
  int rc = MVR_OK;
  for (int a = 0; a < count && rc == MVR_OK; ++a) {
    mvr_ctx* m = ctxs[a];
    if (m != ctx && m->stream != S) {
      if (cudaEventRecord(ev, m->stream) != cudaSuccess || cudaStreamWaitEvent(S, ev, 0) != cudaSuccess) rc = fail(ctx, MVR_ERR_CUDA, "stream ordering failed");
    }
    if (rc) break;
    Cloud& t = m->tgt;
    if (t.gen == 0) { statuses[a] = fail(m, MVR_ERR_NO_INPUT, "target not set"); continue; }
    statuses[a] = MVR_OK;
    if (t.n == 0) continue;
    uint32_t cells = 0;
    const PairGrid g = normals_grid(m, t, k, &cells);
    BuildJob bj;
    m->nq.valid = false;
    if ((rc = plan_pair_index(m, m->nq, 1, t.pts, t.n, t.n_bad, nullptr, g, cells, false, S, &bj))) { ctx->err = m->err; break; }
    if (m->normals.ensure((size_t)t.n * sizeof(float4)) != cudaSuccess) { rc = fail(ctx, MVR_ERR_CUDA, "normals buffer allocation failed"); break; }
    builds.push_back(bj);
    todo.push_back(Todo{m, a, normals_job(m->nq, t.n, viewpoints ? viewpoints + 3 * a : nullptr, m->normals.as<float4>(), nullptr)});
  }
  if (rc == MVR_OK) rc = run_pair_builds(ctx, builds.data(), (int)builds.size(), S);
  for (size_t t0 = 0; rc == MVR_OK && t0 < todo.size(); t0 += BUILD_MAX_JOBS) {
    const int c = (int)std::min(todo.size() - t0, (size_t)BUILD_MAX_JOBS);
    NormalsBatch batch;
    double pts = 0;
    for (int a = 0; a < c; ++a) { batch.j[a] = todo[t0 + a].job; pts += todo[t0 + a].job.n; }
    ProfScope ps(ctx, MVR_K_NORMALS, 32.0 * pts, pts, 1, S);
    const cudaError_t e = launch_normals(batch, c, k, S);
    if (e != cudaSuccess) rc = fail(ctx, MVR_ERR_CUDA, (std::string("launch_normals: ") + cudaGetErrorString(e)).c_str());
  }
  bool copies = false;
  for (size_t a = 0; rc == MVR_OK && a < todo.size(); ++a) {
    mvr_ctx* m = todo[a].m;
    m->nq.valid = false;
    m->has_normals = true;
    float* out = out_nxyzc ? out_nxyzc[todo[a].slot] : nullptr;
    if (!out) continue;
    if (cudaMemcpyAsync(out, m->normals.p, (size_t)m->tgt.n * sizeof(float4), cudaMemcpyDeviceToHost, S) != cudaSuccess) rc = fail(ctx, MVR_ERR_CUDA, "normals copy failed");
    copies = true;
  }
  if (cudaEventRecord(ev, S) == cudaSuccess) {
    for (int a = 0; a < count; ++a) if (ctxs[a]->stream != S) cudaStreamWaitEvent(ctxs[a]->stream, ev, 0);
  } else if (rc == MVR_OK) {
    rc = fail(ctx, MVR_ERR_CUDA, "stream ordering failed");
  }
  ctx->ev_pool.push_back(ev);
  if (rc == MVR_OK && copies) CK(cudaStreamSynchronize(S));
  return rc;
}

}
```

multi-view-registration_b200/csrc/icp.cu:

```cuda
#include <algorithm>

#include "launch.h"
#include "pair_search.cuh"
#ifdef MVR_TS_TILE
#include "tile_search.cuh"
#endif
#include "small_solve.h"

#ifndef MVR_FWD_MINBLOCKS
#define MVR_FWD_MINBLOCKS 5
#endif
#ifndef MVR_FWD1_MINBLOCKS
#define MVR_FWD1_MINBLOCKS 3
#endif
#ifndef MVR_REV_MINBLOCKS
#define MVR_REV_MINBLOCKS 4
#endif
#ifndef MVR_PG_UNROLL
#define MVR_PG_UNROLL 6
#endif

namespace mvr {

template <int NV, int WARPS = 8>
__device__ __forceinline__ void block_reduce_store(double (&v)[NV], double* __restrict__ partials) {
  __shared__ double sm[WARPS][NV];
  const int lane = threadIdx.x & 31, warp = threadIdx.x >> 5;
#pragma unroll
  for (int a = 0; a < NV; ++a) {
    double x = v[a];
#pragma unroll
    for (int o = 16; o > 0; o >>= 1) x += __shfl_down_sync(0xffffffffu, x, o);
    if (lane == 0) sm[warp][a] = x;
  }
  __syncthreads();
  if (threadIdx.x < NV) {
    double x = 0;
#pragma unroll
    for (int w = 0; w < WARPS; ++w) x += sm[w][threadIdx.x];
    partials[(size_t)blockIdx.x * REDUCE_MAX_VALS + threadIdx.x] = x;
  }
}

__device__ __forceinline__ bool last_block_done(unsigned int* ticket, unsigned int nblk) {
  __shared__ bool is_last;
  __threadfence();
  __syncthreads();
  if (threadIdx.x == 0) {
    unsigned int t = atomicAdd(ticket, 1u);
    is_last = (t == nblk - 1);
    if (is_last) *ticket = 0;
  }
  __syncthreads();
  if (is_last) __threadfence();
  return is_last;
}

template <int NV>
__device__ __forceinline__ void ordered_total(const double* __restrict__ partials, int nblk, double* __restrict__ out) {
  __shared__ double ch[FUSED_WARPS][REDUCE_MAX_VALS];
  const int a = threadIdx.x & 31, c = threadIdx.x >> 5;
  const int per = (nblk + FUSED_WARPS - 1) / FUSED_WARPS;
  if (a < NV) {
    const int b0 = c * per, b1 = min(b0 + per, nblk);
    double x = 0;
    int b = b0;
    for (; b + 8 <= b1; b += 8) {
      double t[8];
#pragma unroll
      for (int u = 0; u < 8; ++u) t[u] = __ldcg(partials + (size_t)(b + u) * REDUCE_MAX_VALS + a);
#pragma unroll
      for (int u = 0; u < 8; ++u) x += t[u];
    }
    for (; b < b1; ++b) x += __ldcg(partials + (size_t)b * REDUCE_MAX_VALS + a);
    ch[c][a] = x;
  }
  __syncthreads();
  if (threadIdx.x < NV) {
    double x = 0;
#pragma unroll
    for (int k = 0; k < FUSED_WARPS; ++k) x += ch[k][threadIdx.x];
    out[threadIdx.x] = x;
  }
  __syncthreads();
}

__device__ __forceinline__ void icp_advance_frame(IcpState* st, const double (&Td)[16]) {
  double C0[16], C[16];
#pragma unroll
  for (int k = 0; k < 16; ++k) C0[k] = st->cum[k];
#pragma unroll
  for (int c = 0; c < 4; ++c)
#pragma unroll
    for (int r = 0; r < 4; ++r) {
      double x = 0;
#pragma unroll
      for (int k = 0; k < 4; ++k) x += Td[k * 4 + r] * C0[c * 4 + k];
      C[c * 4 + r] = x;
    }
#pragma unroll
  for (int k = 0; k < 16; ++k) st->cum[k] = C[k];
  const double a00 = C[0], a10 = C[1], a20 = C[2], a01 = C[4], a11 = C[5], a21 = C[6], a02 = C[8], a12 = C[9], a22 = C[10];
  const double c00 = a11 * a22 - a12 * a21, c01 = a12 * a20 - a10 * a22, c02 = a10 * a21 - a11 * a20;
  const double det = a00 * c00 + a01 * c01 + a02 * c02;
  const double id = 1.0 / det;
  double I[9];
  I[0] = c00 * id; I[1] = (a02 * a21 - a01 * a22) * id; I[2] = (a01 * a12 - a02 * a11) * id;
  I[3] = c01 * id; I[4] = (a00 * a22 - a02 * a20) * id; I[5] = (a02 * a10 - a00 * a12) * id;
  I[6] = c02 * id; I[7] = (a01 * a20 - a00 * a21) * id; I[8] = (a00 * a11 - a01 * a10) * id;
#pragma unroll
  for (int r = 0; r < 3; ++r) {
    st->cinv[r * 4 + 0] = I[r * 3 + 0]; st->cinv[r * 4 + 1] = I[r * 3 + 1]; st->cinv[r * 4 + 2] = I[r * 3 + 2];
    st->cinv[r * 4 + 3] = -(I[r * 3 + 0] * C[12] + I[r * 3 + 1] * C[13] + I[r * 3 + 2] * C[14]);
  }
  double eta2 = 0;
#pragma unroll
  for (int i = 0; i < 3; ++i)
#pragma unroll
    for (int j = 0; j < 3; ++j) {
      const double g = C[i * 4 + 0] * C[j * 4 + 0] + C[i * 4 + 1] * C[j * 4 + 1] + C[i * 4 + 2] * C[j * 4 + 2] - ((i == j) ? 1.0 : 0.0);
      eta2 += g * g;
    }
  const double eta = sqrt(eta2);
  st->stretch = (eta < 0.5 && det > 0) ? (float)(1.0 / sqrt(1.0 - eta)) * 1.000001f + 1.0e-7f : 1.0e6f;
  st->n_gate = 0u;

  const double u4 = 4.1 * 5.9604644775390625e-8;
  double e2 = 0, etaT2 = 0;
#pragma unroll
  for (int r = 0; r < 3; ++r) {
    const double er = u4 * (fabs(Td[r]) * st->babs[0] + fabs(Td[4 + r]) * st->babs[1] + fabs(Td[8 + r]) * st->babs[2] + fabs(Td[12 + r])) + 1.0e-30;
    e2 += er * er;
  }
#pragma unroll
  for (int i = 0; i < 3; ++i)
#pragma unroll
    for (int j = 0; j < 3; ++j) {
      const double g = Td[i * 4 + 0] * Td[j * 4 + 0] + Td[i * 4 + 1] * Td[j * 4 + 1] + Td[i * 4 + 2] * Td[j * 4 + 2] - ((i == j) ? 1.0 : 0.0);
      etaT2 += g * g;
    }
  const double devn = st->devd * sqrt(1.0 + sqrt(etaT2)) * (1.0 + 1.0e-9) + sqrt(e2) * (1.0 + 1.0e-9);
  st->devd = devn;
  st->dev = __double2float_ru(devn) * 1.000001f;
  double bn[3] = {0, 0, 0};
#pragma unroll
  for (int c8 = 0; c8 < 8; ++c8) {
    const double px = st->box[(c8 & 1) ? 3 : 0], py = st->box[(c8 & 2) ? 4 : 1], pz = st->box[(c8 & 4) ? 5 : 2];
#pragma unroll
    for (int r = 0; r < 3; ++r) bn[r] = fmax(bn[r], fabs(C[r] * px + C[4 + r] * py + C[8 + r] * pz + C[12 + r]));
  }
#pragma unroll
  for (int r = 0; r < 3; ++r) st->babs[r] = (bn[r] + devn) * (1.0 + 1.0e-6) + 1.0e-3;
}

__device__ __noinline__ void icp_finish_iteration(IcpState* st, IterRec* log) {
  double S[REDUCE_MAX_VALS], F0[16];
#pragma unroll
  for (int k = 0; k < REDUCE_MAX_VALS; ++k) S[k] = st->sums[k];
#pragma unroll
  for (int k = 0; k < 16; ++k) F0[k] = st->fin[k];
  const bool p2l = st->p2l != 0;
  const double ox = st->ox, oy = st->oy, oz = st->oz;
  const int min_corr = st->min_corr, max_iter = st->max_iter, fixed = st->fixed, iter0 = st->iter;
  const double prev_mse = st->prev_mse, rot_thr = st->rot_thr, trans_thr = st->trans_thr, fit_eps = st->fit_eps;
  const double cnt = p2l ? S[27] : S[0];
  const double d2sum = p2l ? S[28] : S[16];
  st->queries += (unsigned long long)st->n_src + (st->recip ? (unsigned long long)st->n_gate : 0ull);
  const int n_corr = (int)cnt;
  st->n_corr = n_corr;
  if (n_corr < min_corr) { st->reason = 5; st->status = 2; st->done = 1; return; }
  double T[16];
  if (p2l) {
    double A[36], b[6], x[6];
    int k = 0;
    for (int a = 0; a < 6; ++a)
      for (int c = a; c < 6; ++c) { A[a * 6 + c] = S[k]; A[c * 6 + a] = S[k]; ++k; }
    for (int a = 0; a < 6; ++a) b[a] = S[21 + a];
    if (!cholesky_solve6(A, b, x)) { st->reason = 5; st->status = 5; st->done = 1; return; }
    pose_from_6(x, T);
  } else {
    const double inv = 1.0 / cnt;
    const double mu_a[3] = {S[1] * inv, S[2] * inv, S[3] * inv}, mu_b[3] = {S[4] * inv, S[5] * inv, S[6] * inv};
    double Sg[9];
#pragma unroll
    for (int r = 0; r < 3; ++r)
#pragma unroll
      for (int c = 0; c < 3; ++c) Sg[r * 3 + c] = S[7 + r * 3 + c] * inv - mu_b[r] * mu_a[c];
    const double mu_s[3] = {mu_a[0] + ox, mu_a[1] + oy, mu_a[2] + oz};
    const double mu_d[3] = {mu_b[0] + ox, mu_b[1] + oy, mu_b[2] + oz};
    umeyama_rigid(mu_s, mu_d, Sg, T);
  }
  float Tf[16];
#pragma unroll
  for (int k = 0; k < 16; ++k) Tf[k] = (float)T[k];
  Tf[3] = Tf[7] = Tf[11] = 0.f; Tf[15] = 1.f;
  double Td[16], F[16];
#pragma unroll
  for (int k = 0; k < 16; ++k) Td[k] = Tf[k];
#pragma unroll
  for (int c = 0; c < 4; ++c)
#pragma unroll
    for (int r = 0; r < 4; ++r) {
      double x = 0;
#pragma unroll
      for (int k = 0; k < 4; ++k) x += Td[k * 4 + r] * F0[c * 4 + k];
      F[c * 4 + r] = x;
    }
#pragma unroll
  for (int k = 0; k < 16; ++k) { st->fin[k] = F[k]; st->delta[k] = Tf[k]; }
  icp_advance_frame(st, Td);
  const int iter = iter0 + 1;
  st->iter = iter;
  const double cur_mse = d2sum / cnt;
  st->cur_mse = cur_mse;
  if (iter <= ICP_MAX_LOG) {
    IterRec& r = log[iter - 1];
    r.iteration = iter; r.n_corr = n_corr; r.mse = cur_mse;
#pragma unroll
    for (int k = 0; k < 16; ++k) r.delta[k] = Tf[k];
  }
  if (iter >= max_iter) { st->done = 1; st->reason = 1; return; }
  if (!fixed) {
    const double cos_angle = 0.5 * (Td[0] + Td[5] + Td[10] - 1.0);
    const double t2 = Td[12] * Td[12] + Td[13] * Td[13] + Td[14] * Td[14];
    if (cos_angle >= rot_thr && t2 <= trans_thr) { st->done = 1; st->reason = 2; return; }
    if (fabs(cur_mse - prev_mse) < 1e-12) { st->done = 1; st->reason = 3; return; }
    if (fabs(cur_mse - prev_mse) / prev_mse < fit_eps) { st->done = 1; st->reason = 4; return; }
    st->prev_mse = cur_mse;
  }
}


__device__ __forceinline__ void acc_p2p(double (&v)[REDUCE_P2P_VALS], float4 s, float4 t, float d2, double ox, double oy, double oz) {
  const double ax = (double)s.x - ox, ay = (double)s.y - oy, az = (double)s.z - oz;
  const double bx = (double)t.x - ox, by = (double)t.y - oy, bz = (double)t.z - oz;
  v[0] += 1.0;
  v[1] += ax; v[2] += ay; v[3] += az;
  v[4] += bx; v[5] += by; v[6] += bz;
  v[7] += bx * ax; v[8] += bx * ay; v[9] += bx * az;
  v[10] += by * ax; v[11] += by * ay; v[12] += by * az;
  v[13] += bz * ax; v[14] += bz * ay; v[15] += bz * az;
  v[16] += (double)d2;
}

__device__ __forceinline__ void acc_mom(double (&v)[REDUCE_MOM_VALS], float4 s, float4 t, float d2, double ox, double oy, double oz) {
  const double ax = (double)s.x - ox, ay = (double)s.y - oy, az = (double)s.z - oz;
  const double bx = (double)t.x - ox, by = (double)t.y - oy, bz = (double)t.z - oz;
  v[0] += 1.0;
  v[1] += ax; v[2] += ay; v[3] += az;
  v[4] += bx; v[5] += by; v[6] += bz;
  v[7] += bx * ax; v[8] += bx * ay; v[9] += bx * az;
  v[10] += by * ax; v[11] += by * ay; v[12] += by * az;
  v[13] += bz * ax; v[14] += bz * ay; v[15] += bz * az;
  v[16] += (double)d2;
  v[17] += ax * ax; v[18] += ax * ay; v[19] += ax * az; v[20] += ay * ay; v[21] += ay * az; v[22] += az * az;
  v[23] += bx * bx; v[24] += bx * by; v[25] += bx * bz; v[26] += by * by; v[27] += by * bz; v[28] += bz * bz;
}

__device__ __forceinline__ void acc_p2l(double (&v)[REDUCE_P2L_VALS], float4 s, float4 t, float4 nn, float d2) {
  const double sx = s.x, sy = s.y, sz = s.z, nx = nn.x, ny = nn.y, nz = nn.z;
  const double J[6] = {nz * sy - ny * sz, nx * sz - nz * sx, ny * sx - nx * sy, nx, ny, nz};
  const double r = nx * ((double)t.x - sx) + ny * ((double)t.y - sy) + nz * ((double)t.z - sz);
  int k = 0;
#pragma unroll
  for (int a = 0; a < 6; ++a)
#pragma unroll
    for (int b = a; b < 6; ++b) v[k++] += J[a] * J[b];
#pragma unroll
  for (int a = 0; a < 6; ++a) v[21 + a] += J[a] * r;
  v[27] += 1.0;
  v[28] += (double)d2;
}

template <int NV>
__device__ __forceinline__ bool block_reduce_ticket(double (&v)[NV], double* __restrict__ partials, unsigned int* ticket, unsigned int nblk) {
  __shared__ double sm[FUSED_WARPS][NV];
  __shared__ bool is_last;
  const int lane = threadIdx.x & 31, warp = threadIdx.x >> 5;
#pragma unroll
  for (int a = 0; a < NV; ++a) {
    double x = v[a];
#pragma unroll
    for (int o = 16; o > 0; o >>= 1) x += __shfl_down_sync(0xffffffffu, x, o);
    if (lane == 0) sm[warp][a] = x;
  }
  __syncthreads();
  if (warp == 0) {
    static_assert(NV <= 32, "one warp writes the partial");
    if (lane < NV) {
      double x = 0;
#pragma unroll
      for (int w = 0; w < FUSED_WARPS; ++w) x += sm[w][lane];
      partials[(size_t)blockIdx.x * REDUCE_MAX_VALS + lane] = x;
      __threadfence();
    }
    __syncwarp();
    if (lane == 0) {
      const unsigned int t = atomicAdd(ticket, 1u);
      is_last = (t == nblk - 1);
      if (is_last) *ticket = 0;
    }
  }
  __syncthreads();
  if (is_last) __threadfence();
  return is_last;
}

template <int NV>
__device__ __forceinline__ void reduce_and_finish(double (&v)[NV], double* __restrict__ partials, IcpState* __restrict__ st,
                                                  IterRec* __restrict__ log, int nblk) {
  if (!block_reduce_ticket<NV>(v, partials, &st->ticket, (unsigned int)nblk)) return;
  ordered_total<NV>(partials, nblk, st->sums);
  if (threadIdx.x == 0) {
    const long long t0 = clock64();
    icp_finish_iteration(st, log);
    st->dbg[0] += clock64() - t0; st->dbg[1] += 1;
  }
}

template <int EST> struct EstVals { static constexpr int value = EST == EST_P2L ? (int)REDUCE_P2L_VALS : (EST == EST_MOM ? (int)REDUCE_MOM_VALS : (int)REDUCE_P2P_VALS); };

template <int EST, int NV>
__device__ __forceinline__ void acc_pair(double (&v)[NV], float4 s, float4 t, const float4* __restrict__ nrm, float d2, double ox, double oy, double oz) {
  if constexpr (EST == EST_P2L) acc_p2l(v, s, t, __ldg(nrm + __float_as_int(t.w)), d2);
  else if constexpr (EST == EST_MOM) acc_mom(v, s, t, d2, ox, oy, oz);
  else acc_p2p(v, s, t, d2, ox, oy, oz);
}

__device__ __forceinline__ void fwd_seed(const FwdArgs& a, int i, const float4 p, NnBest& b) {
  b = NnBest{MVR_INF, 0x7fffffff, -1};
  const int j0 = a.corr_p[i];
  if (j0 >= 0) {
    const float4 t = __ldg(a.tgt + j0);
    b.d2 = d2_pinned(p.x, p.y, p.z, t.x, t.y, t.z); b.idx = __float_as_int(t.w); b.pos = j0;
  }
}

template <bool RECIP>
__device__ __forceinline__ void fwd_commit(const FwdArgs& a, int i, const NnBest& b, unsigned int& ngate) {
  const bool keep = b.pos >= 0 && !((double)b.d2 > a.max2);
  a.corr_p[i] = keep ? b.pos : -1;
  if (keep) {
    ++ngate;
    if (RECIP) atomicMin(a.rmin + b.pos, __float_as_uint(b.d2));
  }
}

#ifdef MVR_TS_TILE
#include "icp_tile.cuh"
#else
template <bool RECIP, int EST>
__global__ void __launch_bounds__(FUSED_THREADS, (RECIP ? MVR_FWD_MINBLOCKS : MVR_FWD1_MINBLOCKS) * (256 / FUSED_THREADS)) k_icp_forward(const __grid_constant__ FwdBatch batch, int first) {
  __shared__ FwdArgs s_args;
  static_assert(sizeof(FwdArgs) % 4 == 0 && sizeof(FwdArgs) / 4 <= FUSED_THREADS, "argument block");
  if (threadIdx.x < sizeof(FwdArgs) / 4) ((uint32_t*)&s_args)[threadIdx.x] = ((const uint32_t*)&batch.a[blockIdx.y])[threadIdx.x];
  __syncthreads();
  const FwdArgs& a = s_args;
  if ((int)blockIdx.x >= a.grid) return;
  IcpState* __restrict__ st = a.st;
  if (st->done) return;
  const int stride = a.grid * FUSED_THREADS;
  __shared__ uint2 s_seg[PG_SEGS * PG_STRIDE];
  uint2* seg = s_seg + threadIdx.x;
  Mat4f M;
  if (!first) {
#pragma unroll
    for (int k = 0; k < 16; ++k) M.m[k] = st->delta[k];
  }
  unsigned int ngate = 0;
  for (int i = blockIdx.x * FUSED_THREADS + threadIdx.x; i < a.n_valid; i += stride) {
    float4 p = a.cur[i];
    if (!first) {
      const float w = p.w;
      p = xform_pinned(M, p);
      p.w = w;
      a.cur[i] = p;
    }
    NnBest b;
    fwd_seed(a, i, p, b);
    if (a.gmask && !(b.d2 <= a.max_d2f)) {
      const int cx = pg_cell(grid_t(p.x, a.gt.ox, a.gt.inv_cell_x), a.gt.nx), cy = pg_cell(grid_t(p.y, a.gt.oy, a.gt.inv_cell), a.gt.ny),
                cz = pg_cell(grid_t(p.z, a.gt.oz, a.gt.inv_cell), a.gt.nz);
      const uint32_t wd = __ldg(a.gmask + ((size_t)cz * a.gt.ny + cy) * a.gm_stride + (cx >> 5));
      if (!((wd >> (cx & 31)) & 1u)) { a.corr_p[i] = -1; continue; }
    }
    pg_search<MVR_PG_UNROLL>(a.gt, a.tstart, a.tgt, a.m_valid, p.x, p.y, p.z, p.x, p.y, p.z, 0.0f, 1.0f, a.max_d2f, b, seg);
    fwd_commit<RECIP>(a, i, b, ngate);
  }
  if (RECIP) {
    const unsigned int wg = __reduce_add_sync(0xffffffffu, ngate);
    if ((threadIdx.x & 31) == 0 && wg) atomicAdd(&st->n_gate, wg);
  } else {
    const double ox = st->ox, oy = st->oy, oz = st->oz;
    constexpr int NV = EstVals<EST>::value;
    double v[NV];
#pragma unroll
    for (int k = 0; k < NV; ++k) v[k] = 0.0;
    for (int i = blockIdx.x * FUSED_THREADS + threadIdx.x; i < a.n_valid; i += stride) {
      const int j = a.corr_p[i];
      if (j < 0) continue;
      const float4 p = a.cur[i];
      const float4 t = __ldg(a.tgt + j);
      acc_pair<EST>(v, p, t, a.nrm, d2_pinned(p.x, p.y, p.z, t.x, t.y, t.z), ox, oy, oz);
    }
    reduce_and_finish<NV>(v, a.partials, st, a.log, a.grid);
  }
}

#ifndef MVR_REV_MAX_CHUNKS
#define MVR_REV_MAX_CHUNKS 4
#endif
constexpr int REV_MAX_CHUNKS = MVR_REV_MAX_CHUNKS;
template <int EST>
__global__ void __launch_bounds__(FUSED_THREADS, MVR_REV_MINBLOCKS * (256 / FUSED_THREADS)) k_icp_reverse(const __grid_constant__ RevBatch batch) {
  __shared__ RevArgs s_args;
  static_assert(sizeof(RevArgs) % 4 == 0 && sizeof(RevArgs) / 4 <= FUSED_THREADS, "argument block");
  if (threadIdx.x < sizeof(RevArgs) / 4) ((uint32_t*)&s_args)[threadIdx.x] = ((const uint32_t*)&batch.a[blockIdx.y])[threadIdx.x];
  __syncthreads();
  const RevArgs& a = s_args;
  if ((int)blockIdx.x >= a.grid) return;
  IcpState* __restrict__ st = a.st;
  if (st->done) return;
  __shared__ uint2 s_seg[PG_SEGS * PG_STRIDE];
  __shared__ int s_q[REV_MAX_CHUNKS * FUSED_THREADS];
  __shared__ int s_p[REV_MAX_CHUNKS * FUSED_THREADS];
  __shared__ int s_wcnt[FUSED_WARPS];
  uint2* seg = s_seg + threadIdx.x;
  const int lane = threadIdx.x & 31, warp = threadIdx.x >> 5;

  const int chunks = (a.m_valid + FUSED_THREADS - 1) / FUSED_THREADS;
  int qn = 0;
  for (int cc = 0; cc < a.per; ++cc) {
    const int c = blockIdx.x * a.per + cc;
    if (c >= chunks) break;
    const int j = c * FUSED_THREADS + threadIdx.x;
    uint32_t r = 0x7f800000u;
    if (j < a.m_valid) {
      r = a.rmin[j];
      if (r != 0x7f800000u) a.rmin[j] = 0x7f800000u;
    }
    const bool chosen = r != 0x7f800000u;
    const unsigned int bal = __ballot_sync(0xffffffffu, chosen);
    if (lane == 0) s_wcnt[warp] = __popc(bal);
    __syncthreads();
    int ofs = qn, tot = 0;
#pragma unroll
    for (int w = 0; w < FUSED_WARPS; ++w) { const int n = s_wcnt[w]; if (w < warp) ofs += n; tot += n; }
    if (chosen) { const int k = ofs + __popc(bal & ((1u << lane) - 1u)); s_q[k] = j; s_p[k] = (int)r; }
    qn += tot;
    __syncthreads();
  }

  const float stretch = st->stretch;
  const float dev0 = st->dev;
  unsigned int missed = 0;
  for (int k = threadIdx.x; k < qn; k += FUSED_THREADS) {
    const int j = s_q[k];
    const float4 t = __ldg(a.tgt + j);
    const float ux = (float)(st->cinv[0] * t.x + st->cinv[1] * t.y + st->cinv[2] * t.z + st->cinv[3]);
    const float uy = (float)(st->cinv[4] * t.x + st->cinv[5] * t.y + st->cinv[6] * t.z + st->cinv[7]);
    const float uz = (float)(st->cinv[8] * t.x + st->cinv[9] * t.y + st->cinv[10] * t.z + st->cinv[11]);
    const float dev = dev0 + 1.0e-6f * fmaxf(fabsf(ux), fmaxf(fabsf(uy), fabsf(uz)));
    NnBest b{__uint_as_float((uint32_t)s_p[k]), 0x7fffffff, -1};
    pg_search<MVR_PG_UNROLL>(a.gs, a.sstart, a.cur, a.n_valid, t.x, t.y, t.z, ux, uy, uz, dev, stretch, MVR_INF, b, seg);
    if (b.pos < 0) ++missed;
    const int mutual = (b.pos >= 0 && __ldg(a.corr_p + b.pos) == j) ? b.pos : -1;
    s_p[k] = mutual;
    if (a.rnn) a.rnn[j] = mutual;
  }
  if (missed) atomicAdd((unsigned long long*)&st->dbg[2], (unsigned long long)missed);

  const double ox = st->ox, oy = st->oy, oz = st->oz;
  constexpr int NV = EstVals<EST>::value;
  double v[NV];
#pragma unroll
  for (int k = 0; k < NV; ++k) v[k] = 0.0;
  for (int k = threadIdx.x; k < qn; k += FUSED_THREADS) {
    const int r = s_p[k];
    if (r < 0) continue;
    const float4 t = __ldg(a.tgt + s_q[k]);
    const float4 s = a.cur[r];
    acc_pair<EST>(v, s, t, a.nrm, d2_pinned(t.x, t.y, t.z, s.x, s.y, s.z), ox, oy, oz);
  }
  reduce_and_finish<NV>(v, a.partials, st, a.log, a.grid);
}
#endif

int fused_rev_chunks(int items) {
#ifdef MVR_REV_CHUNKS
  return MVR_REV_CHUNKS;
#else
#ifdef MVR_TS_TILE
  (void)items;
  return 2;
#else
  return items >= 400000 ? 4 : 3;
#endif
#endif
}
int fused_grid_rev(int items) {
  const int chunks = (items + FUSED_THREADS - 1) / FUSED_THREADS;
  const int per = fused_rev_chunks(items);
  const int blocks = (chunks + per - 1) / per;
  return blocks < 1 ? 1 : blocks;
}

int fused_grid(int items) {
  const int blocks = (items + FUSED_THREADS - 1) / FUSED_THREADS;
  return blocks < 1 ? 1 : (blocks > FUSED_MAX_BLOCKS ? FUSED_MAX_BLOCKS : blocks);
}

#ifdef MVR_SMEM_CARVEOUT
static void set_carveout_once() {
  static bool done = false;
  if (done) return;
  done = true;
  cudaFuncSetAttribute(k_icp_forward<true, EST_P2P>, cudaFuncAttributePreferredSharedMemoryCarveout, MVR_SMEM_CARVEOUT);
  cudaFuncSetAttribute(k_icp_reverse<EST_P2P>, cudaFuncAttributePreferredSharedMemoryCarveout, MVR_SMEM_CARVEOUT);
}
#else
static void set_carveout_once() {}
#endif

cudaError_t launch_icp_forward(const FwdBatch& d_batch, int pairs, int max_grid, int first, bool reciprocal, int est, cudaStream_t s) {
  if (pairs <= 0 || pairs > FUSED_MAX_PAIRS) return pairs <= 0 ? cudaSuccess : cudaErrorInvalidValue;
  set_carveout_once();
  const dim3 grid((unsigned)max_grid, (unsigned)pairs);
  if (reciprocal) {
    k_icp_forward<true, EST_P2P><<<grid, FUSED_THREADS, 0, s>>>(d_batch, first);
  } else {
    if (est == EST_P2L) k_icp_forward<false, EST_P2L><<<grid, FUSED_THREADS, 0, s>>>(d_batch, first);
    else if (est == EST_MOM) k_icp_forward<false, EST_MOM><<<grid, FUSED_THREADS, 0, s>>>(d_batch, first);
    else k_icp_forward<false, EST_P2P><<<grid, FUSED_THREADS, 0, s>>>(d_batch, first);
  }
  count_launch();
  return cudaGetLastError();
}

cudaError_t launch_icp_reverse(const RevBatch& d_batch, int pairs, int max_grid, int est, cudaStream_t s) {
  if (pairs <= 0 || pairs > FUSED_MAX_PAIRS) return pairs <= 0 ? cudaSuccess : cudaErrorInvalidValue;
  const dim3 grid((unsigned)max_grid, (unsigned)pairs);
  if (est == EST_P2L) k_icp_reverse<EST_P2L><<<grid, FUSED_THREADS, 0, s>>>(d_batch);
  else if (est == EST_MOM) k_icp_reverse<EST_MOM><<<grid, FUSED_THREADS, 0, s>>>(d_batch);
  else k_icp_reverse<EST_P2P><<<grid, FUSED_THREADS, 0, s>>>(d_batch);
  count_launch();
  return cudaGetLastError();
}

template <bool BY_W>
__global__ void __launch_bounds__(FUSED_THREADS, 4) k_pair_nn(const float4* __restrict__ q, int n, const float4* __restrict__ tgt,
                                                              const uint32_t* __restrict__ tstart, PairGrid g, int m_valid,
                                                              int32_t* __restrict__ out_idx, float* __restrict__ out_d2) {
  __shared__ uint2 s_seg[PG_SEGS * PG_STRIDE];
  const int i = blockIdx.x * FUSED_THREADS + threadIdx.x;
  if (i >= n) return;
  const float4 p = __ldg(q + i);
  NnBest b{MVR_INF, 0x7fffffff, -1};
  if (finite3(p)) pg_search<MVR_PG_UNROLL>(g, tstart, tgt, m_valid, p.x, p.y, p.z, p.x, p.y, p.z, 0.0f, 1.0f, MVR_INF, b, s_seg + threadIdx.x);
  const int o = BY_W ? __float_as_int(p.w) : i;
  out_idx[o] = b.pos >= 0 ? b.idx : -1;
  out_d2[o] = b.pos >= 0 ? b.d2 : MVR_INF;
}

cudaError_t launch_pair_nn(const float4* q, int n, bool by_w, const float4* tgt_sorted, const uint32_t* tstart, PairGrid g, int m_valid,
                           int32_t* out_idx, float* out_d2, cudaStream_t s) {
  if (n <= 0) return cudaSuccess;
  const int blocks = (n + FUSED_THREADS - 1) / FUSED_THREADS;
  if (by_w) k_pair_nn<true><<<blocks, FUSED_THREADS, 0, s>>>(q, n, tgt_sorted, tstart, g, m_valid, out_idx, out_d2);
  else k_pair_nn<false><<<blocks, FUSED_THREADS, 0, s>>>(q, n, tgt_sorted, tstart, g, m_valid, out_idx, out_d2);
  count_launch();
  return cudaGetLastError();
}

__global__ void __launch_bounds__(256) k_align_init(const __grid_constant__ InitBatch b, const IcpState* __restrict__ stage) {
  const InitJob& j = b.j[blockIdx.y];
  int32_t* __restrict__ corr_p = j.corr_p;
  uint32_t* __restrict__ rmin = j.rmin;
  const int n = j.n, m = rmin ? j.m : 0;
  const int stride = gridDim.x * blockDim.x;
  for (int i = blockIdx.x * blockDim.x + threadIdx.x; i < n; i += stride) corr_p[i] = -1;
  for (int i = blockIdx.x * blockDim.x + threadIdx.x; i < m; i += stride) rmin[i] = 0x7f800000u;
  if (blockIdx.x == 0) {
    static_assert(sizeof(IcpState) % 4 == 0, "IcpState words");
    const uint32_t* src = reinterpret_cast<const uint32_t*>(stage + blockIdx.y);
    uint32_t* dst = reinterpret_cast<uint32_t*>(j.st);
    for (int k = threadIdx.x; k < (int)(sizeof(IcpState) / 4); k += blockDim.x) dst[k] = src[k];
  }
}

__global__ void __launch_bounds__(256) k_align_gather(const __grid_constant__ InitBatch b, IcpState* __restrict__ stage) {
  const InitJob& j = b.j[blockIdx.x];
  const uint32_t* src = reinterpret_cast<const uint32_t*>(j.st);
  uint32_t* dst = reinterpret_cast<uint32_t*>(stage + blockIdx.x);
  for (int k = threadIdx.x; k < (int)(sizeof(IcpState) / 4); k += blockDim.x) dst[k] = src[k];
  __syncthreads();
  if (threadIdx.x == 0) {
    stage[blockIdx.x].dbg[3] = j.crowded ? (long long)*j.crowded : 0ll;
    if (j.crowded) *j.crowded = 0u;
  }
}

cudaError_t launch_align_init(const InitBatch& batch, int count, const IcpState* stage, cudaStream_t s) {
  if (count <= 0) return cudaSuccess;
  if (count > BUILD_MAX_JOBS) return cudaErrorInvalidValue;
  int items = 1;
  for (int k = 0; k < count; ++k) items = std::max(items, std::max(batch.j[k].n, batch.j[k].rmin ? batch.j[k].m : 0));
  const int blocks = std::max(1, std::min((items + 1023) / 1024, (148 * 8 + count - 1) / count));
  k_align_init<<<dim3((unsigned)blocks, (unsigned)count), 256, 0, s>>>(batch, stage); count_launch();
  return cudaGetLastError();
}

cudaError_t launch_align_gather(const InitBatch& batch, int count, IcpState* stage, cudaStream_t s) {
  if (count <= 0) return cudaSuccess;
  if (count > BUILD_MAX_JOBS) return cudaErrorInvalidValue;
  k_align_gather<<<(unsigned)count, 256, 0, s>>>(batch, stage); count_launch();
  return cudaGetLastError();
}

__global__ void k_reduce_final(const double* __restrict__ partials, int nblk, int nv, double* __restrict__ out) {
  int t = threadIdx.x;
  if (t >= nv) return;
  double x = 0;
#pragma unroll 8
  for (int b = 0; b < nblk; ++b) x += partials[(size_t)b * REDUCE_MAX_VALS + t];
  out[t] = x;
}

__global__ void __launch_bounds__(256) k_reduce_fitness(const int32_t* __restrict__ idx, const float* __restrict__ d2, int n,
                                                        double max_range, double* __restrict__ partials) {
  double v[2] = {0.0, 0.0};
  for (int i = blockIdx.x * blockDim.x + threadIdx.x; i < n; i += gridDim.x * blockDim.x) {
    float d = __ldg(d2 + i);
    if (__ldg(idx + i) >= 0 && (double)d <= max_range) { v[0] += (double)d; v[1] += 1.0; }
  }
  block_reduce_store<2>(v, partials);
}

__global__ void __launch_bounds__(256) k_transform_final(const float4* __restrict__ in, float4* __restrict__ out, int n,
                                                         const IcpState* __restrict__ st) {
  int i = blockIdx.x * blockDim.x + threadIdx.x;
  if (i >= n) return;
  Mat4f M;
#pragma unroll
  for (int k = 0; k < 16; ++k) M.m[k] = (float)st->fin[k];
  float4 p = __ldg(in + i);
  out[i] = finite3(p) ? xform_pinned(M, p) : p;
}

cudaError_t launch_transform_final(const float4* in, float4* out, int n, const IcpState* st, cudaStream_t s) {
  if (n <= 0) return cudaSuccess;
  k_transform_final<<<(n + 255) / 256, 256, 0, s>>>(in, out, n, st); count_launch();
  return cudaGetLastError();
}

cudaError_t launch_reduce_fitness(const int32_t* idx, const float* d2, int n, double max_range, double* partials,
                                  double* out, cudaStream_t s) {
  k_reduce_fitness<<<REDUCE_BLOCKS, 256, 0, s>>>(idx, d2, n, max_range, partials); count_launch();
  k_reduce_final<<<1, 32, 0, s>>>(partials, REDUCE_BLOCKS, 2, out); count_launch();
  return cudaGetLastError();
}

__global__ void __launch_bounds__(256) k_resolve_pairs(const float4* __restrict__ src, int n_valid, const int32_t* __restrict__ corr_p,
                                                       const int32_t* __restrict__ rnn, const float4* __restrict__ tgt,
                                                       int32_t* __restrict__ corr_j, float* __restrict__ corr_d2) {
  const int i = blockIdx.x * blockDim.x + threadIdx.x;
  if (i >= n_valid) return;
  const int p = __ldg(corr_p + i);
  if (p < 0 || (rnn && __ldg(rnn + p) != i)) return;
  const float4 s = __ldg(src + i), t = __ldg(tgt + p);
  const int o = __float_as_int(s.w);
  corr_j[o] = __float_as_int(t.w);
  corr_d2[o] = d2_pinned(s.x, s.y, s.z, t.x, t.y, t.z);
}

cudaError_t launch_resolve_pairs(const float4* src_sorted, int n_valid, const int32_t* corr_p, const int32_t* rnn, const float4* tgt_sorted,
                                 int32_t* corr_j, float* corr_d2, cudaStream_t s) {
  if (n_valid <= 0) return cudaSuccess;
  k_resolve_pairs<<<(n_valid + 255) / 256, 256, 0, s>>>(src_sorted, n_valid, corr_p, rnn, tgt_sorted, corr_j, corr_d2); count_launch();
  return cudaGetLastError();
}

constexpr int CP_THREADS = 256;
constexpr int CP_ITEMS = 4;
constexpr int CP_TILE = CP_THREADS * CP_ITEMS;

size_t compact_scratch_elems(int n) { return (size_t)(n > 0 ? (n + CP_TILE - 1) / CP_TILE : 1) + 1; }

__device__ __forceinline__ uint32_t block_excl_scan_256(uint32_t v, uint32_t* total) {
  __shared__ uint32_t ws[8];
  const int lane = threadIdx.x & 31, warp = threadIdx.x >> 5;
  uint32_t incl = v;
#pragma unroll
  for (int o = 1; o < 32; o <<= 1) {
    uint32_t t = __shfl_up_sync(0xffffffffu, incl, o);
    if (lane >= o) incl += t;
  }
  if (lane == 31) ws[warp] = incl;
  __syncthreads();
  uint32_t base = 0, tot = 0;
#pragma unroll
  for (int w = 0; w < 8; ++w) { uint32_t c = ws[w]; if (w < warp) base += c; tot += c; }
  *total = tot;
  __syncthreads();
  return base + incl - v;
}

__global__ void __launch_bounds__(CP_THREADS) k_compact_count(const int32_t* __restrict__ corr_j, int n, uint32_t* __restrict__ counts) {
  int base = blockIdx.x * CP_TILE + threadIdx.x * CP_ITEMS;
  uint32_t c = 0;
#pragma unroll
  for (int a = 0; a < CP_ITEMS; ++a) if (base + a < n && __ldg(corr_j + base + a) >= 0) ++c;
  uint32_t tot;
  block_excl_scan_256(c, &tot);
  if (threadIdx.x == 0) counts[blockIdx.x] = tot;
}

__global__ void __launch_bounds__(1024) k_compact_scan(uint32_t* __restrict__ counts, int nblk, uint32_t* __restrict__ total_out) {
  __shared__ uint32_t ws[32];
  __shared__ uint32_t carry;
  if (threadIdx.x == 0) carry = 0;
  __syncthreads();
  const int lane = threadIdx.x & 31, warp = threadIdx.x >> 5;
  for (int b0 = 0; b0 < nblk; b0 += 1024) {
    int i = b0 + threadIdx.x;
    uint32_t v = i < nblk ? counts[i] : 0, incl = v;
#pragma unroll
    for (int o = 1; o < 32; o <<= 1) {
      uint32_t t = __shfl_up_sync(0xffffffffu, incl, o);
      if (lane >= o) incl += t;
    }
    if (lane == 31) ws[warp] = incl;
    __syncthreads();
    uint32_t base = carry;
    for (int w = 0; w < warp; ++w) base += ws[w];
    if (i < nblk) counts[i] = base + incl - v;
    __syncthreads();
    if (threadIdx.x == 1023) carry = base + incl;
    __syncthreads();
  }
  if (threadIdx.x == 0) { counts[nblk] = carry; *total_out = carry; }
}

__global__ void __launch_bounds__(CP_THREADS) k_compact_write(const int32_t* __restrict__ corr_j, const float* __restrict__ corr_d2,
                                                              int n, const uint32_t* __restrict__ offsets, int32_t* __restrict__ out_q,
                                                              int32_t* __restrict__ out_m, float* __restrict__ out_d2) {
  int base = blockIdx.x * CP_TILE + threadIdx.x * CP_ITEMS;
  int32_t j[CP_ITEMS];
  uint32_t c = 0;
#pragma unroll
  for (int a = 0; a < CP_ITEMS; ++a) { j[a] = (base + a < n) ? __ldg(corr_j + base + a) : -1; if (j[a] >= 0) ++c; }
  uint32_t tot;
  uint32_t pos = offsets[blockIdx.x] + block_excl_scan_256(c, &tot);
#pragma unroll
  for (int a = 0; a < CP_ITEMS; ++a)
    if (j[a] >= 0) { out_q[pos] = base + a; out_m[pos] = j[a]; out_d2[pos] = __ldg(corr_d2 + base + a); ++pos; }
}

cudaError_t launch_compact_corr(const int32_t* corr_j, const float* corr_d2, int n, uint32_t* scratch, int32_t* out_q,
                                int32_t* out_m, float* out_d2, uint32_t* count_out, cudaStream_t s) {
  int nblk = n > 0 ? (n + CP_TILE - 1) / CP_TILE : 0;
  if (nblk > 0) { k_compact_count<<<nblk, CP_THREADS, 0, s>>>(corr_j, n, scratch); count_launch(); }
  k_compact_scan<<<1, 1024, 0, s>>>(scratch, nblk, count_out); count_launch();
  if (nblk > 0) { k_compact_write<<<nblk, CP_THREADS, 0, s>>>(corr_j, corr_d2, n, scratch, out_q, out_m, out_d2); count_launch(); }
  return cudaGetLastError();
}

}
```

multi-view-registration_b200/csrc/launch.h:

```cpp
#pragma once
#include <cuda_runtime.h>
#include <stdint.h>

#include "common.cuh"

namespace mvr {

void count_launch(int n = 1);
unsigned long long launch_count();

cudaError_t launch_bbox_init(uint32_t* out7, cudaStream_t s);
cudaError_t launch_bbox(const float4* pts, int n, uint32_t* out7, cudaStream_t s);
float bbox_decode(uint32_t enc);
struct BboxJob { const float4* pts; int n; int pad_; };
enum { BBOX_MAX_JOBS = 64 };
struct BboxBatch { BboxJob j[BBOX_MAX_JOBS]; };
cudaError_t launch_bbox_batch(const BboxBatch& batch, int count, uint32_t* out7, cudaStream_t s);

cudaError_t launch_apply_pose(const void* in, size_t stride, int n, const double* M16, float4* out, cudaStream_t s);

cudaError_t launch_morton_keys(const float4* pts, int n, GridDev g, uint32_t* keys, uint32_t* vals, cudaStream_t s);
cudaError_t launch_transform_keys(float4* pts, int n, Mat4f M, GridDev g, uint32_t* keys, uint32_t* vals, cudaStream_t s);
cudaError_t launch_transform(const float4* in, float4* out, int n, Mat4f M, cudaStream_t s);

struct SortScratch {
  uint32_t* keys_alt;
  uint32_t* vals_alt;
  uint32_t* hist;
};
int radix_num_blocks(int n);
cudaError_t launch_radix_sort(uint32_t* keys, uint32_t* vals, int n, int key_bits, SortScratch sc, uint32_t** keys_out,
                              uint32_t** vals_out, cudaStream_t s);

cudaError_t launch_gather_sorted(const float4* pts, const uint32_t* perm, int n, float4* sorted, cudaStream_t s);
cudaError_t launch_cell_table(const uint32_t* sorted_keys, int n, int bits, uint32_t* start, cudaStream_t s);

cudaError_t launch_transform_bin(float4* pts, int n, const float* d_delta, const int* d_done, GridDev g, uint32_t* keys,
                                 uint32_t* rank, uint32_t* counters, cudaStream_t s);
int scan_num_tiles(size_t len);
cudaError_t launch_scan_cells(uint32_t* counters, uint32_t* start, size_t len, unsigned long long* tile_state, uint32_t epoch,
                              const int* d_done, cudaStream_t s);
cudaError_t launch_bin_scatter(const float4* pts, int n, const uint32_t* keys, const uint32_t* rank, const uint32_t* start,
                               const int* d_done, float4* sorted, cudaStream_t s);

enum { REDUCE_P2P_VALS = 18, REDUCE_P2L_VALS = 30, REDUCE_MOM_VALS = 30, REDUCE_MAX_VALS = 32, REDUCE_BLOCKS = 592, ICP_MAX_LOG = 1024 };

struct IterRec {
  int iteration;
  int n_corr;
  double mse;
  float delta[16];
};

struct IcpState {
  float delta[16];
  double fin[16];
  double sums[REDUCE_MAX_VALS];
  double prev_mse, cur_mse;
  double rot_thr, trans_thr, fit_eps;
  double ox, oy, oz;
  unsigned long long queries;
  int iter, done, reason, status, n_corr;
  int max_iter, fixed, min_corr, p2l, recip, n_src;
  unsigned int ticket;
  long long dbg[8];
  double cum[16];
  double cinv[12];
  float stretch;
  float dev;
  unsigned int n_gate;
  double devd;
  double box[6];
  double babs[3];
};

#ifndef MVR_FUSED_THREADS
#define MVR_FUSED_THREADS 256
#endif
enum { FUSED_THREADS = MVR_FUSED_THREADS, FUSED_WARPS = FUSED_THREADS / 32, FUSED_MAX_BLOCKS = 148 * 8 * (256 / FUSED_THREADS) };

struct BuildJob {
  const float4* in;
  int n, apply;
  Mat4f M;
  PairGrid g;
  uint32_t cells;
  uint32_t* keys;
  uint32_t* rank;
  uint32_t* counters;
  unsigned long long* tiles;
  uint32_t epoch;
  int ntiles;
  float4* tmp;
  float4* sorted;
  uint32_t* start;
  uint32_t* crowded;
  int ordered;
  int pad_;
};
enum { BUILD_MAX_JOBS = 48 };
struct BuildBatch { BuildJob j[BUILD_MAX_JOBS]; };
cudaError_t launch_pair_builds(const BuildBatch& batch, int count, cudaStream_t s);
cudaError_t launch_scan_cells_batch(const BuildBatch& batch, int count, int max_tiles, cudaStream_t s);
cudaError_t launch_gate_mask(const uint32_t* start, PairGrid g, int wstride, int D, int Dx, uint32_t* occ, uint32_t* mask, cudaStream_t s);
struct FwdArgs {
  float4* cur;
  int n_valid;
  const float4* tgt;
  const uint32_t* tstart;
  PairGrid gt;
  int m_valid;
  int32_t* corr_p;
  uint32_t* rmin;
  double max2;
  float max_d2f;
  const uint32_t* gmask;
  int gm_stride;
  const float4* nrm;
  double* partials;
  IcpState* st;
  IterRec* log;
  int grid;
};
struct RevArgs {
  const float4* tgt;
  int m_valid;
  uint32_t* rmin;
  const float4* cur;
  const uint32_t* sstart;
  PairGrid gs;
  int n_valid;
  const int32_t* corr_p;
  int32_t* rnn;
  const float4* nrm;
  double* partials;
  IcpState* st;
  IterRec* log;
  int grid;
  int per;
};
enum { EST_P2P = 0, EST_P2L = 1, EST_MOM = 2  };
enum { FUSED_MAX_PAIRS = 24 };
struct FwdBatch { FwdArgs a[FUSED_MAX_PAIRS]; };
struct RevBatch { RevArgs a[FUSED_MAX_PAIRS]; };
struct InitJob { int32_t* corr_p; int n; int m; uint32_t* rmin; IcpState* st; uint32_t* crowded; };
struct InitBatch { InitJob j[BUILD_MAX_JOBS]; };
cudaError_t launch_align_init(const InitBatch& batch, int count, const IcpState* stage, cudaStream_t s);
cudaError_t launch_align_gather(const InitBatch& batch, int count, IcpState* stage, cudaStream_t s);
int fused_grid(int items);
int fused_grid_rev(int items);
int fused_rev_chunks(int items);
cudaError_t launch_icp_forward(const FwdBatch& batch, int pairs, int max_grid, int first, bool reciprocal, int est, cudaStream_t s);
cudaError_t launch_icp_reverse(const RevBatch& batch, int pairs, int max_grid, int est, cudaStream_t s);
cudaError_t launch_pair_nn(const float4* q, int n, bool by_w, const float4* tgt_sorted, const uint32_t* tstart, PairGrid g, int m_valid,
                           int32_t* out_idx, float* out_d2, cudaStream_t s);
cudaError_t launch_resolve_pairs(const float4* src_sorted, int n_valid, const int32_t* corr_p, const int32_t* rnn, const float4* tgt_sorted,
                                 int32_t* corr_j, float* corr_d2, cudaStream_t s);
cudaError_t launch_transform_final(const float4* in, float4* out, int n, const IcpState* st, cudaStream_t s);
cudaError_t launch_reduce_fitness(const int32_t* idx, const float* d2, int n, double max_range, double* partials,
                                  double* out, cudaStream_t s);

size_t compact_scratch_elems(int n);
cudaError_t launch_compact_corr(const int32_t* corr_j, const float* corr_d2, int n, uint32_t* scratch, int32_t* out_q,
                                int32_t* out_m, float* out_d2, uint32_t* count_out, cudaStream_t s);

cudaError_t launch_merge_rich(const void* in48, int n, const double* M16, int full_matrix_normals, void* out48, cudaStream_t s);

cudaError_t launch_cell_nn(const float4* q_sorted, int nq, const uint32_t* d_nq_valid, const float4* tgt_sorted, const uint32_t* tstart,
                           PairGrid g, int m_valid, int32_t* out_idx, float* out_d2, cudaStream_t s);

cudaError_t launch_seeded_nn(const float4* q_sorted, int nq, const uint32_t* d_nq_valid, const float4* tgt_sorted, const uint32_t* tstart,
                             PairGrid g, int m_valid, int32_t* out_idx, float* out_d2, cudaStream_t s);

cudaError_t launch_warp_nn(const float4* q, int n, const float4* tgt_sorted, const uint32_t* tstart, PairGrid g, int m_valid, int32_t* out_idx,
                           float* out_d2, cudaStream_t s);

cudaError_t launch_denoise_components(const float4* sorted, const uint32_t* start, PairGrid g, int n, int n_valid, double threshold,
                                      uint32_t* parent, uint32_t* root, uint32_t* count, cudaStream_t s);
cudaError_t launch_denoise_keys(const uint32_t* count, int n, uint32_t segment_threshold, uint32_t* keys, uint32_t* vals,
                                uint32_t* n_noise, cudaStream_t s);

struct NormalsJob {
  const float4* sorted;
  const uint32_t* start;
  PairGrid g;
  int n, n_valid;
  float3 viewpoint;
  float4* out;
  int32_t* nbr;
};
struct NormalsBatch { NormalsJob j[BUILD_MAX_JOBS]; };
cudaError_t launch_normals(const NormalsBatch& batch, int count, int k, cudaStream_t s);

}
```

multi-view-registration_b200/csrc/pair_index.cu:

```cuda
#include <algorithm>

#include "launch.h"
#include "pair_search.cuh"

namespace mvr {

__device__ __forceinline__ const BuildJob& load_job(const BuildBatch& b, BuildJob& s_job) {
  static_assert(sizeof(BuildJob) % 4 == 0 && sizeof(BuildJob) / 4 <= 256, "job block");
  if (threadIdx.x < sizeof(BuildJob) / 4) ((uint32_t*)&s_job)[threadIdx.x] = ((const uint32_t*)&b.j[blockIdx.y])[threadIdx.x];
  __syncthreads();
  return s_job;
}

__global__ void __launch_bounds__(256) k_pair_count(const __grid_constant__ BuildBatch b) {
  __shared__ BuildJob s_job;
  const BuildJob& j = load_job(b, s_job);
  const int i = blockIdx.x * blockDim.x + threadIdx.x;
  if (i >= j.n) return;
  float4 p = __ldg(j.in + i);
  const bool ok = finite3(p);
  if (j.apply && ok) p = xform_pinned(j.M, p);
  const uint32_t key = ok ? pg_key(p, j.g) : j.cells;
  j.keys[i] = key;
  j.rank[i] = atomicAdd(j.counters + key, 1u);
}

__global__ void __launch_bounds__(256) k_pair_scatter(const __grid_constant__ BuildBatch b) {
  __shared__ BuildJob s_job;
  const BuildJob& j = load_job(b, s_job);
  const int i = blockIdx.x * blockDim.x + threadIdx.x;
  if (i >= j.n) return;
  float4 p = __ldg(j.in + i);
  if (j.apply && finite3(p)) p = xform_pinned(j.M, p);
  p.w = __uint_as_float((uint32_t)i);
  (j.ordered ? j.tmp : j.sorted)[__ldg(j.start + __ldg(j.keys + i)) + __ldg(j.rank + i)] = p;
}

constexpr uint32_t RERANK_LIMIT = 1024;
__global__ void __launch_bounds__(256) k_pair_rerank(const __grid_constant__ BuildBatch b) {
  __shared__ BuildJob s_job;
  const BuildJob& j = load_job(b, s_job);
  const int k = blockIdx.x * blockDim.x + threadIdx.x;
  if (k >= j.n || !j.ordered) return;
  const float4* __restrict__ tmp = j.tmp;
  const float4 p = __ldg(tmp + k);
  const uint32_t idx = __float_as_uint(p.w);
  const uint32_t key = __ldg(j.keys + idx);
  const uint32_t s = __ldg(j.start + key), e = __ldg(j.start + key + 1);
  if (e - s > RERANK_LIMIT) {
    j.sorted[k] = p;
    if (j.crowded && (uint32_t)k == s) atomicMax(j.crowded, e - s);
    return;
  }
  uint32_t r = 0;
  for (uint32_t q = s; q < e; ++q) r += (__float_as_uint(__ldg(&tmp[q].w)) < idx) ? 1u : 0u;
  j.sorted[s + r] = p;
}

__global__ void __launch_bounds__(256) k_gate_occ(const uint32_t* __restrict__ start, PairGrid g, int wstride, size_t words, uint32_t* __restrict__ occ) {
  const size_t w = (size_t)blockIdx.x * blockDim.x + threadIdx.x;
  if (w >= words) return;
  const size_t row = w / (size_t)wstride;
  const int xw = (int)(w % (size_t)wstride);
  const uint32_t* r = start + row * (size_t)g.nx;
  uint32_t bits = 0;
  uint32_t prev = __ldg(r + xw * 32);
  for (int b = 0; b < 32; ++b) {
    const int x = xw * 32 + b;
    if (x >= g.nx) break;
    const uint32_t next = __ldg(r + x + 1);
    if (next > prev) bits |= 1u << b;
    prev = next;
  }
  occ[w] = bits;
}

__global__ void __launch_bounds__(256) k_gate_dilate(const uint32_t* __restrict__ occ, PairGrid g, int wstride, int D, int Dx, size_t words, uint32_t* __restrict__ out) {
  const size_t w = (size_t)blockIdx.x * blockDim.x + threadIdx.x;
  if (w >= words) return;
  const int xw = (int)(w % (size_t)wstride);
  const size_t row = w / (size_t)wstride;
  const int y = (int)(row % (size_t)g.ny), z = (int)(row / (size_t)g.ny);
  uint32_t acc = 0;
  for (int zz = max(z - D, 0); zz <= min(z + D, g.nz - 1); ++zz)
    for (int yy = max(y - D, 0); yy <= min(y + D, g.ny - 1); ++yy) {
      const uint32_t* r = occ + ((size_t)zz * g.ny + yy) * wstride;
      const uint32_t cur = __ldg(r + xw), prev = xw > 0 ? __ldg(r + xw - 1) : 0u, next = xw + 1 < wstride ? __ldg(r + xw + 1) : 0u;
      uint32_t v = cur;
      for (int k = 1; k <= Dx; ++k) v |= (cur << k) | (cur >> k) | (prev >> (32 - k)) | (next << (32 - k));
      acc |= v;
    }
  out[w] = acc;
}

cudaError_t launch_gate_mask(const uint32_t* start, PairGrid g, int wstride, int D, int Dx, uint32_t* occ, uint32_t* mask, cudaStream_t s) {
  const size_t words = (size_t)g.ny * g.nz * wstride;
  if (words == 0 || D < 1 || Dx < 1 || Dx > 31) return cudaErrorInvalidValue;
  const unsigned blocks = (unsigned)((words + 255) / 256);
  k_gate_occ<<<blocks, 256, 0, s>>>(start, g, wstride, words, occ); count_launch();
  k_gate_dilate<<<blocks, 256, 0, s>>>(occ, g, wstride, D, Dx, words, mask); count_launch();
  return cudaGetLastError();
}

cudaError_t launch_pair_builds(const BuildBatch& batch, int count, cudaStream_t s) {
  if (count <= 0) return cudaSuccess;
  if (count > BUILD_MAX_JOBS) return cudaErrorInvalidValue;
  int max_n = 0, max_tiles = 0;
  bool any_ordered = false;
  for (int k = 0; k < count; ++k) {
    max_n = std::max(max_n, batch.j[k].n);
    max_tiles = std::max(max_tiles, batch.j[k].ntiles);
    any_ordered = any_ordered || batch.j[k].ordered;
  }
  const dim3 gp((unsigned)std::max((max_n + 255) / 256, 1), (unsigned)count);
  if (max_n > 0) { k_pair_count<<<gp, 256, 0, s>>>(batch); count_launch(); }
  launch_scan_cells_batch(batch, count, max_tiles, s);
  if (max_n > 0) { k_pair_scatter<<<gp, 256, 0, s>>>(batch); count_launch(); }
  if (max_n > 0 && any_ordered) { k_pair_rerank<<<gp, 256, 0, s>>>(batch); count_launch(); }
  return cudaGetLastError();
}

}
```

Baseline: 14.82 billion.

## Share per-view grid indices across pair contexts and apply guess in init

```diff
diff --git a/multi-view-registration_b200/csrc/api.cu b/multi-view-registration_b200/csrc/api.cu
--- a/multi-view-registration_b200/csrc/api.cu
+++ b/multi-view-registration_b200/csrc/api.cu
@@ -1,3 +1,4 @@
+#include <algorithm>
 #include <cfloat>
 #include <chrono>
 #include <cstdlib>
@@ -5,6 +6,7 @@
 #include <cmath>
 #include <cstdio>
 #include <cstring>
+#include <atomic>
 #include <memory>
 #include <string>
 #include <thread>
@@ -20,7 +22,6 @@
 
 using namespace mvr;
 
-#include <atomic>
 namespace mvr {
 static std::atomic<unsigned long long> g_launches{0};
 void count_launch(int n) { g_launches.fetch_add((unsigned long long)n, std::memory_order_relaxed); }
@@ -45,6 +46,31 @@
   template <class T> T* as() const { return (T*)p; }
 };
 
+struct PairIndex {
+  DevBuf sorted, start;
+  PairGrid g{};
+  uint32_t cells = 0;
+  int n_valid = 0;
+  uint64_t gen = 0;
+  uint64_t owner = 0;
+  bool valid = false;
+  void release() { sorted.release(); start.release(); valid = false; }
+};
+
+std::shared_ptr<PairIndex> new_view_index(int device) {
+  return std::shared_ptr<PairIndex>(new PairIndex, [device](PairIndex* p) {
+    int cur = 0;
+    cudaGetDevice(&cur);
+    cudaSetDevice(device);
+    p->release();
+    cudaSetDevice(cur);
+    delete p;
+  });
+}
+
+std::atomic<uint64_t> g_cloud_gen{0};
+uint64_t next_cloud_gen() { return g_cloud_gen.fetch_add(1, std::memory_order_relaxed) + 1; }
+
 struct Cloud {
   const float4* pts = nullptr;
   DevBuf own;
@@ -52,6 +78,7 @@
   float lo[3] = {0, 0, 0}, hi[3] = {0, 0, 0};
   int n_bad = 0;
   uint64_t gen = 0;
+  std::shared_ptr<PairIndex> ix, own_ix;
   bool index_valid = false;
   bool exportable = false;
   uint64_t index_gen = 0;
@@ -68,23 +95,11 @@
   void release() {
     own.release(); keys.release(); vals.release(); keys_alt.release(); vals_alt.release(); hist.release();
     counters.release(); sorted.release(); table.release();
+    ix.reset(); own_ix.reset();
   }
 };
 
 struct ProfRec { int kind; cudaEvent_t a, b; double bytes, units; int count; };
-
-struct PairIndex {
-  DevBuf sorted, start, s0;
-  DevBuf gocc, gmask;
-  float gm_gate = -1.f;
-  int gm_stride = 0;
-  PairGrid g{};
-  uint32_t cells = 0;
-  int n_valid = 0;
-  uint64_t gen = 0;
-  bool valid = false;
-  void release() { sorted.release(); start.release(); s0.release(); gocc.release(); gmask.release(); gm_gate = -1.f; valid = false; }
-};
 
 }
 
@@ -95,17 +110,25 @@
   Cloud tgt, src;
   DevBuf normals; bool has_normals = false;
   DevBuf cur, corr_p, corr_j, corr_d2, rmin, rnn, partials, sums, out_cloud, qtmp, itmp, ftmp, scratch, misc, tiles, state, log;
-  PairIndex pt, ps;
+  PairIndex pt;
   PairIndex nt, nq;
   double nn_ppc = 8.0;
   double nn_dense_ratio = 8.0;
   int nn_mode = MVR_NN_AUTO;
   int nn_sorted_from = 262144;
   bool gate_mask = false;
+  DevBuf gocc, gmask;
+  float gm_gate = -1.f;
+  int gm_stride = 0;
+  uint64_t gm_gen = 0;
+  PairGrid gm_g{};
   FwdArgs fa{}; RevArgs ra{};
   bool want_rnn = false;
   int group_pairs = 0;
   struct BuildScratch { DevBuf keys, vals, moved, count, tiles; uint32_t epoch = 1; } bs[2];
+  PairGrid plan_gt{}, plan_gs{};
+  uint32_t plan_ct = 0, plan_cs = 0;
+  bool plan_guess = false;
   DevBuf stage_dev;
   IcpState* h_stage = nullptr;
   int stage_cap = 0;
@@ -238,11 +261,18 @@
   return MVR_OK;
 }
 
+void cloud_renew(mvr_ctx* ctx, Cloud& c) {
+  c.index_valid = false;
+  c.gen = next_cloud_gen();
+  if (!c.own_ix) c.own_ix = new_view_index(ctx->device);
+  c.ix = c.own_ix;
+  c.ix->owner = c.gen;
+}
+
 int cloud_set(mvr_ctx* ctx, Cloud& c, const float* xyzw, size_t n, bool device_ptr) {
   if (n > (size_t)INT_MAX / 2) return fail(ctx, MVR_ERR_BAD_ARG, "cloud too large");
   if (n > 0 && !xyzw) return fail(ctx, MVR_ERR_BAD_ARG, "null point pointer");
-  c.index_valid = false;
-  c.gen++;
+  cloud_renew(ctx, c);
   c.n = (int)n;
   if (device_ptr) {
     c.pts = (const float4*)xyzw;
@@ -294,10 +324,9 @@
 
 PairGrid make_pair_grid(const float lo[3], const float hi[3], double e, uint32_t* cells_out, int xr = 1);
 bool same_pair_grid(const PairGrid& a, const PairGrid& b);
-int build_pair_index(mvr_ctx* ctx, PairIndex& ix, const float4* pts, int n, int n_bad, const Mat4f* guess, const PairGrid& g,
-                     uint32_t cells, bool keep_s0, bool ordered = true);
-int plan_pair_index(mvr_ctx* ctx, PairIndex& ix, int slot, const float4* pts, int n, int n_bad, const Mat4f* guess, const PairGrid& g,
-                    uint32_t cells, bool ordered, cudaStream_t stream, BuildJob* job);
+int build_pair_index(mvr_ctx* ctx, PairIndex& ix, const float4* pts, int n, int n_bad, const PairGrid& g, uint32_t cells, bool ordered = true);
+int plan_pair_index(mvr_ctx* ctx, PairIndex& ix, int slot, const float4* pts, int n, int n_bad, const PairGrid& g, uint32_t cells, bool ordered,
+                    cudaStream_t stream, BuildJob* job);
 int run_pair_builds(mvr_ctx* ctx, const BuildJob* jobs, int count, cudaStream_t stream);
 
 double pair_cell_edge(mvr_ctx* ctx, const Cloud& c, double max_dist);
@@ -310,10 +339,10 @@
   const PairGrid g = make_pair_grid(t.lo, t.hi, e, &cells);
   int rc;
   if (!(ctx->nt.valid && ctx->nt.gen == t.gen && same_pair_grid(ctx->nt.g, g))) {
-    if ((rc = build_pair_index(ctx, ctx->nt, t.pts, t.n, t.n_bad, nullptr, g, cells, false))) return rc;
+    if ((rc = build_pair_index(ctx, ctx->nt, t.pts, t.n, t.n_bad, g, cells))) return rc;
     ctx->nt.gen = t.gen;
   }
-  if ((rc = build_pair_index(ctx, ctx->nq, q, n, 0, nullptr, g, cells, false, false))) return rc;
+  if ((rc = build_pair_index(ctx, ctx->nq, q, n, 0, g, cells, false))) return rc;
   ProfScope ps(ctx, MVR_K_NN, 24.0 * n + 16.0 * t.n, (double)n);
   if (seeded)
     CK(launch_seeded_nn(ctx->nq.sorted.as<float4>(), n, ctx->nq.start.as<uint32_t>() + cells, ctx->nt.sorted.as<float4>(),
@@ -333,7 +362,7 @@
   if (!(pt.valid && pt.gen == t.gen && pt.g.xr == 1.0f)) {
     uint32_t cells = 0;
     const PairGrid gt = make_pair_grid(t.lo, t.hi, pair_cell_edge(ctx, t, INFINITY), &cells);
-    if ((rc = build_pair_index(ctx, pt, t.pts, t.n, t.n_bad, nullptr, gt, cells, false))) return rc;
+    if ((rc = build_pair_index(ctx, pt, t.pts, t.n, t.n_bad, gt, cells))) return rc;
     pt.gen = t.gen;
   }
   ProfScope ps(ctx, MVR_K_NN, 24.0 * n + 16.0 * t.n, (double)n);
@@ -342,7 +371,7 @@
     return MVR_OK;
   }
   const bool sorted = n > 262144;
-  if (sorted && (rc = build_pair_index(ctx, ctx->nq, q, n, 0, nullptr, pt.g, pt.cells, false, false))) return rc;
+  if (sorted && (rc = build_pair_index(ctx, ctx->nq, q, n, 0, pt.g, pt.cells, false))) return rc;
   CK(launch_pair_nn(sorted ? ctx->nq.sorted.as<float4>() : q, n, sorted, pt.sorted.as<float4>(), pt.start.as<uint32_t>(), pt.g, pt.n_valid, d_idx,
                     d_d2, ctx->stream));
   return MVR_OK;
@@ -403,8 +432,8 @@
 
 bool same_pair_grid(const PairGrid& a, const PairGrid& b) { return std::memcmp(&a, &b, sizeof(PairGrid)) == 0; }
 
-int plan_pair_index(mvr_ctx* ctx, PairIndex& ix, int slot, const float4* pts, int n, int n_bad, const Mat4f* guess, const PairGrid& g,
-                    uint32_t cells, bool ordered, cudaStream_t stream, BuildJob* job) {
+int plan_pair_index(mvr_ctx* ctx, PairIndex& ix, int slot, const float4* pts, int n, int n_bad, const PairGrid& g, uint32_t cells, bool ordered,
+                    cudaStream_t stream, BuildJob* job) {
   mvr_ctx::BuildScratch& bs = ctx->bs[slot];
   const size_t nn = (size_t)std::max(n, 1);
   CK(bs.keys.ensure(nn * sizeof(uint32_t)));
@@ -425,15 +454,14 @@
   if (!ctx->crowded.p) { CK(ctx->crowded.ensure(64)); CK(cudaMemsetAsync(ctx->crowded.p, 0, 64, stream)); }
   BuildJob& j = *job;
   j = BuildJob{};
-  j.in = pts; j.n = n; j.apply = guess ? 1 : 0;
-  if (guess) j.M = *guess;
+  j.in = pts; j.n = n;
   j.g = g; j.cells = cells;
   j.keys = bs.keys.as<uint32_t>(); j.rank = bs.vals.as<uint32_t>(); j.counters = bs.count.as<uint32_t>();
   j.tiles = bs.tiles.as<unsigned long long>(); j.epoch = bs.epoch; j.ntiles = ntiles;
   bs.epoch = (bs.epoch % 0x3fffffffu) + 1;
   j.tmp = ordered ? bs.moved.as<float4>() : nullptr; j.sorted = ix.sorted.as<float4>(); j.start = ix.start.as<uint32_t>();
   j.crowded = ctx->crowded.as<uint32_t>(); j.ordered = ordered ? 1 : 0;
-  ix.g = g; ix.cells = cells; ix.n_valid = n - n_bad; ix.valid = true; ix.gm_gate = -1.f;
+  ix.g = g; ix.cells = cells; ix.n_valid = n - n_bad; ix.valid = true;
   return MVR_OK;
 }
 
@@ -449,32 +477,30 @@
   return MVR_OK;
 }
 
-int build_pair_index(mvr_ctx* ctx, PairIndex& ix, const float4* pts, int n, int n_bad, const Mat4f* guess, const PairGrid& g,
-                     uint32_t cells, bool keep_s0, bool ordered) {
-  (void)keep_s0;
+int build_pair_index(mvr_ctx* ctx, PairIndex& ix, const float4* pts, int n, int n_bad, const PairGrid& g, uint32_t cells, bool ordered) {
   BuildJob job;
   ix.valid = false;
-  int rc = plan_pair_index(ctx, ix, &ix == &ctx->pt || &ix == &ctx->nt ? 0 : 1, pts, n, n_bad, guess, g, cells, ordered, ctx->stream, &job);
+  int rc = plan_pair_index(ctx, ix, &ix == &ctx->pt || &ix == &ctx->nt ? 0 : 1, pts, n, n_bad, g, cells, ordered, ctx->stream, &job);
   if (rc) { ix.valid = false; return rc; }
   return run_pair_builds(ctx, &job, 1, ctx->stream);
 }
 
-int ensure_gate_mask(mvr_ctx* ctx, PairIndex& ix, float max_d2f, cudaStream_t stream) {
-  if (!ctx->gate_mask || !(max_d2f < 3.0e38f) || ix.n_valid <= 0) { ix.gm_gate = -1.f; return MVR_OK; }
-  if (ix.gm_gate == max_d2f) return MVR_OK;
+int ensure_gate_mask(mvr_ctx* ctx, const PairIndex& ix, float max_d2f, cudaStream_t stream) {
+  if (!ctx->gate_mask || !(max_d2f < 3.0e38f) || ix.n_valid <= 0) { ctx->gm_gate = -1.f; return MVR_OK; }
+  if (ctx->gm_gate == max_d2f && ctx->gm_gen == ix.gen && same_pair_grid(ctx->gm_g, ix.g)) return MVR_OK;
   const double slack = 2.0 * ((double)MVR_CELL_MARGIN + 1.0e-6 * (double)std::max(ix.g.nx, std::max(ix.g.ny, ix.g.nz)));
   const double need = std::sqrt((double)max_d2f) * (1.0 + 1.0e-5) / (double)ix.g.cell_lo + slack;
   const int D = (int)std::ceil(need);
   const int Dx = (int)std::ceil(need * (double)ix.g.xr);
-  ix.gm_gate = -1.f;
+  ctx->gm_gate = -1.f;
   if (D < 1 || D > 6 || Dx > 31) return MVR_OK;
   const int wstride = (ix.g.nx + 31) / 32;
   const size_t words = (size_t)ix.g.ny * ix.g.nz * wstride;
-  CK(ix.gocc.ensure(words * sizeof(uint32_t)));
-  CK(ix.gmask.ensure(words * sizeof(uint32_t)));
-  CK(launch_gate_mask(ix.start.as<uint32_t>(), ix.g, wstride, D, Dx, ix.gocc.as<uint32_t>(), ix.gmask.as<uint32_t>(), stream));
-  ix.gm_stride = wstride;
-  ix.gm_gate = max_d2f;
+  CK(ctx->gocc.ensure(words * sizeof(uint32_t)));
+  CK(ctx->gmask.ensure(words * sizeof(uint32_t)));
+  CK(launch_gate_mask(ix.start.as<uint32_t>(), ix.g, wstride, D, Dx, ctx->gocc.as<uint32_t>(), ctx->gmask.as<uint32_t>(), stream));
+  ctx->gm_stride = wstride;
+  ctx->gm_gate = max_d2f; ctx->gm_gen = ix.gen; ctx->gm_g = ix.g;
   return MVR_OK;
 }
 
@@ -579,13 +605,14 @@
   if (ctx->ev_a) cudaEventDestroy(ctx->ev_a);
   if (ctx->ev_b) cudaEventDestroy(ctx->ev_b);
   ctx->tgt.release(); ctx->src.release(); ctx->normals.release();
-  ctx->pt.release(); ctx->ps.release(); ctx->nt.release(); ctx->nq.release();
+  ctx->pt.release(); ctx->nt.release(); ctx->nq.release();
   for (auto& b : ctx->bs) { b.keys.release(); b.vals.release(); b.moved.release(); b.count.release(); b.tiles.release(); }
   ctx->stage_dev.release(); ctx->bbox_dev.release();
   if (ctx->h_stage) cudaFreeHost(ctx->h_stage);
   if (ctx->h_bbox) cudaFreeHost(ctx->h_bbox);
   DevBuf* bufs[] = {&ctx->cur, &ctx->corr_p, &ctx->rmin, &ctx->rnn, &ctx->corr_j, &ctx->corr_d2, &ctx->partials, &ctx->sums, &ctx->out_cloud, &ctx->qtmp,
-                    &ctx->itmp, &ctx->ftmp, &ctx->scratch, &ctx->misc, &ctx->tiles, &ctx->state, &ctx->log, &ctx->crowded};
+                    &ctx->itmp, &ctx->ftmp, &ctx->scratch, &ctx->misc, &ctx->tiles, &ctx->state, &ctx->log, &ctx->crowded,
+                    &ctx->gocc, &ctx->gmask};
   for (DevBuf* b : bufs) b->release();
   if (ctx->h_sums) cudaFreeHost(ctx->h_sums);
   if (ctx->h_small) cudaFreeHost(ctx->h_small);
@@ -653,7 +680,7 @@
 int mvr_ctx_set_gate_mask(mvr_ctx* ctx, int on) {
   if (!ctx) return MVR_ERR_BAD_ARG;
   ctx->gate_mask = on != 0;
-  ctx->pt.gm_gate = -1.f;
+  ctx->gm_gate = -1.f;
   return MVR_OK;
 }
 
@@ -719,8 +746,7 @@
       mvr_ctx* m = ctxs[k0 + k];
       Cloud& cl = which[k0 + k] == MVR_CLOUD_TARGET ? m->tgt : m->src;
       if (which[k0 + k] == MVR_CLOUD_TARGET) m->has_normals = false; else { m->have_out = false; m->out_pending = false; }
-      cl.index_valid = false;
-      cl.gen++;
+      cloud_renew(m, cl);
       cl.n = (int)n[k0 + k];
       cl.pts = (const float4*)d_xyzw[k0 + k];
       const uint32_t* w = ctx->h_bbox + 7 * k;
@@ -741,8 +767,10 @@
   Cloud& d = which_dst == MVR_CLOUD_TARGET ? dst->tgt : dst->src;
   if (s.gen == 0) return fail(dst, MVR_ERR_NO_INPUT, "cloud not set");
   if (&s == &d) return MVR_OK;
+  cudaSetDevice(dst->device);
   d.index_valid = false;
-  d.gen++;
+  d.gen = s.gen;
+  d.ix = s.ix;
   d.pts = s.pts; d.n = s.n; d.n_bad = s.n_bad;
   for (int a = 0; a < 3; ++a) { d.lo[a] = s.lo[a]; d.hi[a] = s.hi[a]; }
   if (which_dst == MVR_CLOUD_TARGET) dst->has_normals = false; else dst->have_out = false;
@@ -881,7 +909,7 @@
   return MVR_OK;
 }
 
-static int align_plan(mvr_ctx* ctx, const mvr_icp_params* prm, const float* guess, int est, cudaStream_t S, std::vector<BuildJob>& jobs) {
+static int align_plan(mvr_ctx* ctx, const mvr_icp_params* prm, const float* guess, int est) {
   cudaSetDevice(ctx->device);
   if (ctx->tgt.gen == 0 || ctx->src.gen == 0) return fail(ctx, MVR_ERR_NO_INPUT, "source/target not set");
   Cloud& s = ctx->src;
@@ -897,42 +925,10 @@
   const bool p2l = est == EST_P2L;
 
   const int m = ctx->tgt.n;
-  int rc = MVR_OK;
-  {
-    uint32_t cells = 0;
-    const PairGrid gt = make_pair_grid(ctx->tgt.lo, ctx->tgt.hi, pair_cell_edge(ctx, ctx->tgt, max_dist), &cells, MVR_PG_XRATIO);
-    PairIndex& pt = ctx->pt;
-    if (!(pt.valid && pt.gen == ctx->tgt.gen && same_pair_grid(pt.g, gt))) {
-      BuildJob job;
-      pt.valid = false;
-      if ((rc = plan_pair_index(ctx, pt, 0, ctx->tgt.pts, m, ctx->tgt.n_bad, nullptr, gt, cells, true, S, &job))) { pt.valid = false; return rc; }
-      jobs.push_back(job);
-      pt.gen = ctx->tgt.gen;
-    }
-  }
-  {
-    float lo[3] = {INFINITY, INFINITY, INFINITY}, hi[3] = {-INFINITY, -INFINITY, -INFINITY};
-    if (s.n - s.n_bad > 0) {
-      for (int corner = 0; corner < 8; ++corner) {
-        const double p[3] = {(corner & 1) ? s.hi[0] : s.lo[0], (corner & 2) ? s.hi[1] : s.lo[1], (corner & 4) ? s.hi[2] : s.lo[2]};
-        for (int a = 0; a < 3; ++a) {
-          const double v = G[a] * p[0] + G[4 + a] * p[1] + G[8 + a] * p[2] + G[12 + a];
-          if (std::isfinite(v)) { lo[a] = std::min(lo[a], (float)v); hi[a] = std::max(hi[a], (float)v); }
-        }
-      }
-    }
-    for (int a = 0; a < 3; ++a) if (!(lo[a] <= hi[a])) { lo[a] = 0.f; hi[a] = 0.f; }
-    uint32_t cells = 0;
-    const PairGrid gs = make_pair_grid(lo, hi, pair_cell_edge(ctx, s, max_dist), &cells, MVR_PG_XRATIO);
-    Mat4f Gm;
-    std::memcpy(Gm.m, G, sizeof(Gm.m));
-    BuildJob job;
-    ctx->ps.valid = false;
-    if ((rc = plan_pair_index(ctx, ctx->ps, 1, s.pts, n, s.n_bad, &Gm, gs, cells, true, S, &job))) { ctx->ps.valid = false; return rc; }
-    jobs.push_back(job);
-    for (int a = 0; a < 3; ++a) { ctx->h_state->box[a] = lo[a]; ctx->h_state->box[3 + a] = hi[a]; }
-  }
-  const PairIndex &pt = ctx->pt, &psx = ctx->ps;
+  ctx->plan_gt = make_pair_grid(ctx->tgt.lo, ctx->tgt.hi, pair_cell_edge(ctx, ctx->tgt, max_dist), &ctx->plan_ct, MVR_PG_XRATIO);
+  ctx->plan_gs = make_pair_grid(s.lo, s.hi, pair_cell_edge(ctx, s, max_dist), &ctx->plan_cs, MVR_PG_XRATIO);
+  ctx->plan_guess = guess != nullptr;
+  CK(ctx->cur.ensure((size_t)std::max(n, 1) * sizeof(float4)));
   CK(ctx->corr_p.ensure((size_t)std::max(n, 1) * sizeof(int32_t)));
   if (reciprocal) CK(ctx->rmin.ensure((size_t)std::max(m, 1) * sizeof(uint32_t)));
   CK(ctx->partials.ensure((size_t)std::max((int)FUSED_MAX_BLOCKS, fused_grid_rev(m)) * REDUCE_MAX_VALS * sizeof(double)));
@@ -942,12 +938,10 @@
   IterRec* d_log = ctx->log.as<IterRec>();
 
   IcpState& h = *ctx->h_state;
-  double sbox[6];
-  for (int a = 0; a < 6; ++a) sbox[a] = h.box[a];
   std::memset(&h, 0, sizeof(h));
   for (int a = 0; a < 3; ++a) {
-    const double pad = 1e-3 + 1e-5 * std::max(std::fabs(sbox[a]), std::fabs(sbox[3 + a]));
-    h.box[a] = sbox[a] - pad; h.box[3 + a] = sbox[3 + a] + pad;
+    const double pad = 1e-3 + 1e-5 * std::max(std::fabs((double)s.lo[a]), std::fabs((double)s.hi[a]));
+    h.box[a] = (double)s.lo[a] - pad; h.box[3 + a] = (double)s.hi[a] + pad;
     h.babs[a] = std::max(std::fabs(h.box[a]), std::fabs(h.box[3 + a]));
   }
   h.devd = 0.0; h.dev = 0.0f;
@@ -970,23 +964,57 @@
   ctx->log_pending = 0;
   ctx->have_out = false; ctx->out_pending = false;
 
+  const int n_valid = n - s.n_bad, m_valid = m - ctx->tgt.n_bad;
   FwdArgs& fa = ctx->fa;
   fa = FwdArgs{};
-  fa.cur = psx.sorted.as<float4>(); fa.n_valid = psx.n_valid;
-  fa.tgt = pt.sorted.as<float4>(); fa.tstart = pt.start.as<uint32_t>(); fa.gt = pt.g; fa.m_valid = pt.n_valid;
+  fa.cur = ctx->cur.as<float4>(); fa.n_valid = n_valid;
+  fa.gt = ctx->plan_gt; fa.m_valid = m_valid;
   fa.corr_p = ctx->corr_p.as<int32_t>(); fa.rmin = reciprocal ? ctx->rmin.as<uint32_t>() : nullptr;
   fa.max2 = max_dist * max_dist; fa.max_d2f = gate_float(max_dist);
   fa.gmask = nullptr; fa.gm_stride = 0;
   fa.nrm = p2l ? ctx->normals.as<float4>() : nullptr;
-  fa.partials = ctx->partials.as<double>(); fa.st = d_st; fa.log = d_log; fa.grid = fused_grid(psx.n_valid);
+  fa.partials = ctx->partials.as<double>(); fa.st = d_st; fa.log = d_log; fa.grid = fused_grid(n_valid);
   RevArgs& ra = ctx->ra;
   ra = RevArgs{};
-  ra.tgt = fa.tgt; ra.m_valid = pt.n_valid; ra.rmin = fa.rmin; ra.cur = fa.cur; ra.sstart = psx.start.as<uint32_t>(); ra.gs = psx.g;
-  ra.n_valid = psx.n_valid; ra.corr_p = fa.corr_p; ra.nrm = fa.nrm;
+  ra.m_valid = m_valid; ra.rmin = fa.rmin; ra.cur = fa.cur; ra.gs = ctx->plan_gs;
+  ra.n_valid = n_valid; ra.corr_p = fa.corr_p; ra.nrm = fa.nrm;
   ra.rnn = nullptr;
   if (reciprocal && ctx->want_rnn) { CK(ctx->rnn.ensure((size_t)std::max(m, 1) * sizeof(int32_t))); ra.rnn = ctx->rnn.as<int32_t>(); }
-  ra.partials = fa.partials; ra.st = d_st; ra.log = d_log; ra.grid = fused_grid_rev(pt.n_valid); ra.per = fused_rev_chunks(pt.n_valid);
-  return MVR_OK;
+  ra.partials = fa.partials; ra.st = d_st; ra.log = d_log; ra.grid = fused_grid_rev(m_valid); ra.per = fused_rev_chunks(m_valid);
+  return MVR_OK;
+}
+
+struct IndexUse { PairIndex* ix; int group; };
+
+static int view_index(mvr_ctx* m, Cloud& c, const PairGrid& g, uint32_t cells, int slot, int group, cudaStream_t S,
+                      std::vector<IndexUse>& used, std::vector<BuildJob>& jobs, std::vector<int>& waits, PairIndex** out) {
+  for (;;) {
+    PairIndex* ix = c.ix.get();
+    int at = -1;
+    for (size_t u = 0; u < used.size(); ++u) if (used[u].ix == ix) at = (int)u;
+    if (ix->valid && ix->gen == c.gen && same_pair_grid(ix->g, g)) {
+      if (at < 0) used.push_back(IndexUse{ix, -1});
+      else if (used[(size_t)at].group >= 0 && used[(size_t)at].group != group) waits.push_back(used[(size_t)at].group);
+      *out = ix;
+      return MVR_OK;
+    }
+    if (at < 0 && ix->owner == c.gen) {
+      BuildJob job;
+      ix->valid = false;
+      const int rc = plan_pair_index(m, *ix, slot, c.pts, c.n, c.n_bad, g, cells, true, S, &job);
+      if (rc) { ix->valid = false; return rc; }
+      ix->gen = c.gen;
+      jobs.push_back(job);
+      used.push_back(IndexUse{ix, group});
+      *out = ix;
+      return MVR_OK;
+    }
+    bool own_free = c.own_ix && c.own_ix.get() != ix;
+    for (const IndexUse& u : used) own_free = own_free && u.ix != c.own_ix.get();
+    if (!own_free) c.own_ix = new_view_index(m->device);
+    c.ix = c.own_ix;
+    c.ix->owner = c.gen;
+  }
 }
 
 static int ensure_stage(mvr_ctx* lead, int count) {
@@ -1017,51 +1045,66 @@
                                std::vector<mvr_ctx*>& ok, std::vector<int>& slot) {
   ok.clear(); slot.clear();
   if (count <= 0) return MVR_OK;
-  const int gsz0 = batch_group_size(ctxs[0], count);
-  std::vector<std::vector<BuildJob>> jobs((size_t)count);
   for (int k = 0; k < count; ++k) if (ensure_pinned(ctxs[k]) != MVR_OK) return MVR_ERR_CUDA;
-  parallel_for(count, [&](int k) {
-    statuses[k] = align_plan(ctxs[k], prm, guesses ? guesses + 16 * k : nullptr, est, ctxs[(k / gsz0) * gsz0]->stream, jobs[(size_t)k]);
-  });
+  parallel_for(count, [&](int k) { statuses[k] = align_plan(ctxs[k], prm, guesses ? guesses + 16 * k : nullptr, est); });
   for (int k = 0; k < count; ++k)
     if (statuses[k] == MVR_OK) { ok.push_back(ctxs[k]); slot.push_back(k); }
   if (ok.empty()) return MVR_OK;
   mvr_ctx* ctx = ok[0];
   const int P = (int)ok.size();
   const int gsz = batch_group_size(ctx, P);
-  if (P != count || gsz != gsz0) {
-    for (int k = 0; k < count; k += gsz0) {
-      cudaEvent_t e = ctxs[k]->ev_b;
-      CK(cudaEventRecord(e, ctxs[k]->stream));
-      for (int g0 = 0; g0 < P; g0 += gsz) CK(cudaStreamWaitEvent(ok[(size_t)g0]->stream, e, 0));
-    }
-  }
   int rc = ensure_stage(ctx, P);
   if (rc) return rc;
-  for (int g0 = 0; g0 < P; g0 += gsz) {
-    const int gn = std::min(gsz, P - g0);
+  std::vector<IndexUse> used;
+  std::vector<cudaEvent_t> built;
+  auto give_back = [&] { for (cudaEvent_t e : built) if (e) ctx->ev_pool.push_back(e); };
+  for (int g0 = 0; g0 < P && rc == MVR_OK; g0 += gsz) {
+    const int gn = std::min(gsz, P - g0), gi = g0 / gsz;
     cudaStream_t S = ok[(size_t)g0]->stream;
-    std::vector<BuildJob> all;
-    for (int k = 0; k < gn; ++k) { const std::vector<BuildJob>& j = jobs[(size_t)slot[(size_t)(g0 + k)]]; all.insert(all.end(), j.begin(), j.end()); }
-    if ((rc = run_pair_builds(ctx, all.data(), (int)all.size(), S))) return rc;
-    for (int k0 = 0; k0 < gn; k0 += BUILD_MAX_JOBS) {
+    std::vector<BuildJob> jobs;
+    std::vector<int> waits;
+    std::vector<PairIndex*> tix((size_t)gn), six((size_t)gn);
+    for (int k = 0; k < gn && rc == MVR_OK; ++k) {
+      mvr_ctx* m = ok[(size_t)(g0 + k)];
+      rc = view_index(m, m->tgt, m->plan_gt, m->plan_ct, 0, gi, S, used, jobs, waits, &tix[(size_t)k]);
+      if (rc == MVR_OK) rc = view_index(m, m->src, m->plan_gs, m->plan_cs, 1, gi, S, used, jobs, waits, &six[(size_t)k]);
+      if (rc) { ctx->err = m->err; break; }
+      m->fa.tgt = tix[(size_t)k]->sorted.as<float4>(); m->fa.tstart = tix[(size_t)k]->start.as<uint32_t>();
+      m->ra.tgt = m->fa.tgt; m->ra.sstart = six[(size_t)k]->start.as<uint32_t>();
+    }
+    if (rc) break;
+    if ((rc = run_pair_builds(ctx, jobs.data(), (int)jobs.size(), S))) break;
+    built.push_back(nullptr);
+    if (!jobs.empty()) {
+      built.back() = get_event(ctx);
+      if (!built.back()) { rc = fail(ctx, MVR_ERR_CUDA, "cudaEventCreate failed"); break; }
+      if (cudaEventRecord(built.back(), S) != cudaSuccess) { rc = fail(ctx, MVR_ERR_CUDA, "cudaEventRecord failed"); break; }
+    }
+    for (size_t w = 0; w < waits.size() && rc == MVR_OK; ++w)
+      if (std::find(waits.begin(), waits.begin() + w, waits[w]) == waits.begin() + w && cudaStreamWaitEvent(S, built[(size_t)waits[w]], 0) != cudaSuccess)
+        rc = fail(ctx, MVR_ERR_CUDA, "cudaStreamWaitEvent failed");
+    for (int k0 = 0; k0 < gn && rc == MVR_OK; k0 += BUILD_MAX_JOBS) {
       const int c = std::min(gn - k0, (int)BUILD_MAX_JOBS);
       InitBatch ib;
       for (int k = 0; k < c; ++k) {
         mvr_ctx* m = ok[(size_t)(g0 + k0 + k)];
         ib.j[k] = init_job_of(m);
+        ib.j[k].src = six[(size_t)(k0 + k)]->sorted.as<float4>(); ib.j[k].cur = m->cur.as<float4>(); ib.j[k].guess = m->plan_guess ? 1 : 0;
         std::memcpy(ctx->h_stage + g0 + k0 + k, m->h_state, sizeof(IcpState));
       }
-      CK(cudaMemcpyAsync(ctx->stage_dev.as<IcpState>() + g0 + k0, ctx->h_stage + g0 + k0, (size_t)c * sizeof(IcpState), cudaMemcpyHostToDevice, S));
-      CK(launch_align_init(ib, c, ctx->stage_dev.as<IcpState>() + g0 + k0, S));
+      if (cudaMemcpyAsync(ctx->stage_dev.as<IcpState>() + g0 + k0, ctx->h_stage + g0 + k0, (size_t)c * sizeof(IcpState), cudaMemcpyHostToDevice, S) != cudaSuccess ||
+          launch_align_init(ib, c, ctx->stage_dev.as<IcpState>() + g0 + k0, S) != cudaSuccess)
+        rc = fail(ctx, MVR_ERR_CUDA, "align initialisation failed");
     }
-    for (int k = 0; k < gn; ++k) {
+    for (int k = 0; k < gn && rc == MVR_OK; ++k) {
       mvr_ctx* m = ok[(size_t)(g0 + k)];
-      if ((rc = ensure_gate_mask(m, m->pt, m->fa.max_d2f, S))) { ctx->err = m->err; return rc; }
-      m->fa.gmask = m->pt.gm_gate >= 0.f ? m->pt.gmask.as<uint32_t>() : nullptr; m->fa.gm_stride = m->pt.gm_stride;
+      if ((rc = ensure_gate_mask(m, *tix[(size_t)k], m->fa.max_d2f, S))) { ctx->err = m->err; break; }
+      m->fa.gmask = m->gm_gate >= 0.f ? m->gmask.as<uint32_t>() : nullptr; m->fa.gm_stride = m->gm_stride;
     }
   }
-  return MVR_OK;
+  give_back();
+  if (rc) for (const IndexUse& u : used) if (u.group >= 0) u.ix->valid = false;
+  return rc;
 }
 
 static int align_run(mvr_ctx* const* ctxs, int count, const mvr_icp_params* prm, int est) {
@@ -1487,7 +1530,7 @@
   const PairGrid g = make_pair_grid(tmp.lo, tmp.hi, triangle_length * 1.0001, &cells);
   if ((double)g.cell_lo < triangle_length) return fail(ctx, MVR_ERR_BAD_ARG, "cloud too large for this edge length (grid capped)");
   PairIndex& ix = ctx->nq;
-  if ((rc = build_pair_index(ctx, ix, tmp.pts, ni, tmp.n_bad, nullptr, g, cells, false, false))) return rc;
+  if ((rc = build_pair_index(ctx, ix, tmp.pts, ni, tmp.n_bad, g, cells, false))) return rc;
   const size_t nb = (size_t)radix_num_blocks(ni) * 256;
   CK(ctx->itmp.ensure(((size_t)6 * n + nb + 16) * sizeof(uint32_t)));
   uint32_t* parent = ctx->itmp.as<uint32_t>();
@@ -1520,7 +1563,7 @@
   uint32_t cells = 0;
   const PairGrid g = normals_grid(ctx, c, k, &cells);
   PairIndex& ix = ctx->nq;
-  int rc = build_pair_index(ctx, ix, c.pts, n, c.n_bad, nullptr, g, cells, false, false);
+  int rc = build_pair_index(ctx, ix, c.pts, n, c.n_bad, g, cells, false);
   if (rc) return rc;
   DevBuf& nb = which == MVR_CLOUD_TARGET ? ctx->normals : ctx->qtmp;
   CK(nb.ensure((size_t)n * sizeof(float4)));
@@ -1572,7 +1615,7 @@
     const PairGrid g = normals_grid(m, t, k, &cells);
     BuildJob bj;
     m->nq.valid = false;
-    if ((rc = plan_pair_index(m, m->nq, 1, t.pts, t.n, t.n_bad, nullptr, g, cells, false, S, &bj))) { ctx->err = m->err; break; }
+    if ((rc = plan_pair_index(m, m->nq, 1, t.pts, t.n, t.n_bad, g, cells, false, S, &bj))) { ctx->err = m->err; break; }
     if (m->normals.ensure((size_t)t.n * sizeof(float4)) != cudaSuccess) { rc = fail(ctx, MVR_ERR_CUDA, "normals buffer allocation failed"); break; }
     builds.push_back(bj);
     todo.push_back(Todo{m, a, normals_job(m->nq, t.n, viewpoints ? viewpoints + 3 * a : nullptr, m->normals.as<float4>(), nullptr)});
diff --git a/multi-view-registration_b200/csrc/icp.cu b/multi-view-registration_b200/csrc/icp.cu
--- a/multi-view-registration_b200/csrc/icp.cu
+++ b/multi-view-registration_b200/csrc/icp.cu
@@ -580,11 +580,32 @@
   const int stride = gridDim.x * blockDim.x;
   for (int i = blockIdx.x * blockDim.x + threadIdx.x; i < n; i += stride) corr_p[i] = -1;
   for (int i = blockIdx.x * blockDim.x + threadIdx.x; i < m; i += stride) rmin[i] = 0x7f800000u;
+  const IcpState& s0 = stage[blockIdx.y];
+  Mat4f G;
+#pragma unroll
+  for (int k = 0; k < 16; ++k) G.m[k] = (float)s0.fin[k];
+  const float4* __restrict__ in = j.src;
+  float4* __restrict__ cur = j.cur;
+  for (int i = blockIdx.x * blockDim.x + threadIdx.x; in && i < n; i += stride) {
+    float4 p = __ldg(in + i);
+    if (j.guess && finite3(p)) { const float w = p.w; p = xform_pinned(G, p); p.w = w; }
+    cur[i] = p;
+  }
   if (blockIdx.x == 0) {
     static_assert(sizeof(IcpState) % 4 == 0, "IcpState words");
-    const uint32_t* src = reinterpret_cast<const uint32_t*>(stage + blockIdx.y);
+    const uint32_t* src = reinterpret_cast<const uint32_t*>(&s0);
     uint32_t* dst = reinterpret_cast<uint32_t*>(j.st);
     for (int k = threadIdx.x; k < (int)(sizeof(IcpState) / 4); k += blockDim.x) dst[k] = src[k];
+    if (j.guess) {
+      __syncthreads();
+      if (threadIdx.x == 0) {
+        double Td[16];
+#pragma unroll
+        for (int k = 0; k < 16; ++k) Td[k] = (double)G.m[k];
+        Td[3] = Td[7] = Td[11] = 0.0; Td[15] = 1.0;
+        icp_advance_frame(j.st, Td);
+      }
+    }
   }
 }
 
diff --git a/multi-view-registration_b200/csrc/launch.h b/multi-view-registration_b200/csrc/launch.h
--- a/multi-view-registration_b200/csrc/launch.h
+++ b/multi-view-registration_b200/csrc/launch.h
@@ -81,8 +81,7 @@
 
 struct BuildJob {
   const float4* in;
-  int n, apply;
-  Mat4f M;
+  int n, pad0_;
   PairGrid g;
   uint32_t cells;
   uint32_t* keys;
@@ -143,7 +142,12 @@
 enum { FUSED_MAX_PAIRS = 24 };
 struct FwdBatch { FwdArgs a[FUSED_MAX_PAIRS]; };
 struct RevBatch { RevArgs a[FUSED_MAX_PAIRS]; };
-struct InitJob { int32_t* corr_p; int n; int m; uint32_t* rmin; IcpState* st; uint32_t* crowded; };
+struct InitJob {
+  int32_t* corr_p; int n; int m; uint32_t* rmin; IcpState* st; uint32_t* crowded;
+  const float4* src;
+  float4* cur;
+  int guess, pad_;
+};
 struct InitBatch { InitJob j[BUILD_MAX_JOBS]; };
 cudaError_t launch_align_init(const InitBatch& batch, int count, const IcpState* stage, cudaStream_t s);
 cudaError_t launch_align_gather(const InitBatch& batch, int count, IcpState* stage, cudaStream_t s);
diff --git a/multi-view-registration_b200/csrc/pair_index.cu b/multi-view-registration_b200/csrc/pair_index.cu
--- a/multi-view-registration_b200/csrc/pair_index.cu
+++ b/multi-view-registration_b200/csrc/pair_index.cu
@@ -17,10 +17,8 @@
   const BuildJob& j = load_job(b, s_job);
   const int i = blockIdx.x * blockDim.x + threadIdx.x;
   if (i >= j.n) return;
-  float4 p = __ldg(j.in + i);
-  const bool ok = finite3(p);
-  if (j.apply && ok) p = xform_pinned(j.M, p);
-  const uint32_t key = ok ? pg_key(p, j.g) : j.cells;
+  const float4 p = __ldg(j.in + i);
+  const uint32_t key = finite3(p) ? pg_key(p, j.g) : j.cells;
   j.keys[i] = key;
   j.rank[i] = atomicAdd(j.counters + key, 1u);
 }
@@ -31,7 +29,6 @@
   const int i = blockIdx.x * blockDim.x + threadIdx.x;
   if (i >= j.n) return;
   float4 p = __ldg(j.in + i);
-  if (j.apply && finite3(p)) p = xform_pinned(j.M, p);
   p.w = __uint_as_float((uint32_t)i);
   (j.ordered ? j.tmp : j.sorted)[__ldg(j.start + __ldg(j.keys + i)) + __ldg(j.rank + i)] = p;
 }
```

New measurement: 14.93 billion (median of 6 runs). About the same (+0.8%).
